# elybrand/quantized_neural_networks

Measured on NVIDIA B200. Metric: quantized weights/s, full-network GPFQ pass, higher is better.
Workload: dtype f64

## Files before the change

### quantized_neural_networks_b200/csrc/api.cu

```cuda
#include <math.h>
#include <stdarg.h>
#include <stdlib.h>

#include <algorithm>
#include <cmath>

#include "common.cuh"

int dense_gram_path(gpfq_ctx *, const float *, const float *, int64_t, int64_t, int64_t, const float *, int64_t,
                    int64_t, int64_t, const double *, const int *, const int *, int, double *, int64_t, int64_t,
                    gpfq_stats *, const double *G1_pre = nullptr, const double *G2_pre = nullptr, const double *d_scales = nullptr,
                    int64_t u0 = 0);
int dense_stream_path(gpfq_ctx *, const float *, const float *, int64_t, int64_t, int64_t, const float *, int64_t,
                      int64_t, int64_t, const double *, const int *, const int *, int, double *, int64_t, int64_t,
                      gpfq_stats *, const double *d_scales, int64_t u0);
int dense_gram_only(gpfq_ctx *, const float *, const float *, int64_t, int64_t, int64_t, double *, double *);
bool dense_gram_uses_i8(gpfq_ctx *, int64_t, int64_t, bool);
int conv_supported_kk(int kk);
int conv_pick_chunks(gpfq_ctx *, int64_t, int, int64_t *, int, bool, int64_t part_rows = 0);
bool conv_specialised_kk(int kk);
int conv_gram_stage(gpfq_ctx *, int, ConvPtrs, bool, int64_t, int, int, int64_t, double *, bool, int);
int conv_finalize_stage(gpfq_ctx *, const double *, int, int, int, bool, double *);
int conv_sweep_stage(gpfq_ctx *, int, const double *, const float *, double *, int64_t, int64_t, int64_t, int,
                     const double *, const int *, const int *, int, int64_t, const double *);
int im2col_stage(gpfq_ctx *, const float *, int64_t, int, int, int64_t, int64_t, int, int, int, int, int, int, int,
                 int, int, int, int, float *, int64_t);
int msq_stage(gpfq_ctx *, const void *, int, int64_t, const double *, int, int, double *, const double *, int64_t);
int nhwc9_plan(int, int, int, int, int, int, int, int, int *, int *);
int corr9_plan(int, int, int, int, int, int, int, int, int, int);
int corr9_pack_stage(gpfq_ctx *, const float *, int64_t, int, int, int64_t, int64_t, int, int, int64_t, int64_t, float *);
int corr9_pick_slots(gpfq_ctx *, int, bool, int64_t, int, int64_t, int);
int corr9_uses_strips(gpfq_ctx *, int);
int corr9_tensor_ok(const float *, const float *);
int conv_corr9_stage(gpfq_ctx *, const float *, const float *, bool, int64_t, int64_t, int64_t, int, int, int64_t, int64_t, int,
                     int, double *, int, int, int, double *, int, int, int);
int conv_corr9_assemble_stage(gpfq_ctx *, const double *, int, const double *, int, bool, int, int, double *);
int conv_gram9_nhwc_stage(gpfq_ctx *, const float *, const float *, bool, int64_t, int64_t, int, int, int64_t, int64_t, int,
                          int, int, int, int, int, int, int, double *, int);

int gpfq_fail(gpfq_ctx *ctx, int code, const char *fmt, ...) {
    char buf[1024];
    va_list ap;
    va_start(ap, fmt);
    vsnprintf(buf, sizeof(buf), fmt, ap);
    va_end(ap);
    if (ctx) ctx->err = buf;
    return code;
}

int gpfq_ws(gpfq_ctx *ctx, int slot, size_t bytes, void **out) {
    DevBuf &b = ctx->ws[slot];
    if (bytes == 0) bytes = 16;
    if (b.cap < bytes) {
        if (b.p) {
            CUDA_TRY(ctx, cudaStreamSynchronize(ctx->stream));
            CUDA_TRY(ctx, cudaStreamSynchronize(ctx->copy_stream));
            for (auto &s : ctx->aux_stream) if (s) CUDA_TRY(ctx, cudaStreamSynchronize(s));
            CUDA_TRY(ctx, cudaFree(b.p));
            b.p = nullptr;
            b.cap = 0;
        }
        size_t cap = (bytes + ((size_t)1 << 20) - 1) & ~(((size_t)1 << 20) - 1);
        cudaError_t e = cudaMalloc(&b.p, cap);
        if (e != cudaSuccess) {
            b.p = nullptr;
            cudaGetLastError();
            return gpfq_fail(ctx, GPFQ_ERR_OOM, "cudaMalloc of %zu bytes (workspace %d) failed: %s", cap, slot,
                             cudaGetErrorString(e));
        }
        b.cap = cap;
    }
    *out = b.p;
    return GPFQ_OK;
}

int gpfq_pinned(gpfq_ctx *ctx, int slot, size_t bytes, void **out) {
    DevBuf &b = ctx->pinned[slot];
    if (bytes == 0) bytes = 16;
    if (b.cap < bytes) {
        if (b.p) {
            CUDA_TRY(ctx, cudaStreamSynchronize(ctx->stream));
            CUDA_TRY(ctx, cudaFreeHost(b.p));
            b.p = nullptr;
            b.cap = 0;
        }
        cudaError_t e = cudaMallocHost(&b.p, bytes);
        if (e != cudaSuccess) {
            b.p = nullptr;
            cudaGetLastError();
            return gpfq_fail(ctx, GPFQ_ERR_OOM, "cudaMallocHost of %zu bytes failed: %s", bytes, cudaGetErrorString(e));
        }
        b.cap = bytes;
    }
    *out = b.p;
    return GPFQ_OK;
}

extern "C" int gpfq_version(void) { return GPFQ_VERSION; }

extern "C" int gpfq_create(int device, gpfq_ctx **out) {
    if (!out) return GPFQ_ERR_ARG;
    *out = nullptr;
    int ndev = 0;
    if (cudaGetDeviceCount(&ndev) != cudaSuccess || device < 0 || device >= ndev) {
        cudaGetLastError();
        return GPFQ_ERR_UNSUPPORTED;
    }
    cudaDeviceProp prop;
    if (cudaGetDeviceProperties(&prop, device) != cudaSuccess) return GPFQ_ERR_CUDA;
    if (prop.major != 10) return GPFQ_ERR_UNSUPPORTED;
    if (cudaSetDevice(device) != cudaSuccess) return GPFQ_ERR_CUDA;
    gpfq_ctx *ctx = new gpfq_ctx();
    ctx->device = device;
    ctx->sm_count = prop.multiProcessorCount;
    ctx->smem_optin = prop.sharedMemPerBlockOptin;
    bool ok = cudaStreamCreateWithFlags(&ctx->own_stream, cudaStreamNonBlocking) == cudaSuccess &&
              cudaStreamCreateWithFlags(&ctx->copy_stream, cudaStreamNonBlocking) == cudaSuccess;
    ctx->ring.resize(GPFQ_RING);
    for (auto &r : ctx->ring)
        for (int i = 0; ok && i < 8; ++i) ok = cudaEventCreate(&r.e[i]) == cudaSuccess;
    ctx->cur = &ctx->ring[0];
    for (int i = 0; ok && i < 4; ++i) ok = cudaEventCreateWithFlags(&ctx->ev_copy[i], cudaEventDisableTiming) == cudaSuccess;
    for (int i = 0; ok && i < 12; ++i) ok = cudaEventCreateWithFlags(&ctx->ev_chain[i], cudaEventDisableTiming) == cudaSuccess;
    for (int i = 0; ok && i < 8; ++i) ok = cudaStreamCreateWithFlags(&ctx->aux_stream[i], cudaStreamNonBlocking) == cudaSuccess;
    if (!ok) {
        delete ctx;
        return GPFQ_ERR_CUDA;
    }
    ctx->stream = ctx->own_stream;
    *out = ctx;
    return GPFQ_OK;
}

extern "C" int64_t gpfq_conv_partial_bytes(gpfq_ctx *ctx) { return ctx ? ctx->conv_part_bytes : 0; }

extern "C" int gpfq_trim(gpfq_ctx *ctx) {
    if (!ctx) return GPFQ_ERR_ARG;
    cudaSetDevice(ctx->device);
    cudaStreamSynchronize(ctx->stream);
    cudaStreamSynchronize(ctx->copy_stream);
    for (auto &s : ctx->aux_stream) if (s) cudaStreamSynchronize(s);
    for (auto &b : ctx->ws) {
        if (b.p) cudaFree(b.p);
        b.p = nullptr;
        b.cap = 0;
    }
    for (auto &b : ctx->pinned) {
        if (b.p) cudaFreeHost(b.p);
        b.p = nullptr;
        b.cap = 0;
    }
    ctx->alph_cache.clear();
    ctx->alph_used = 0;
    ctx->i8_oom_bytes = 0;
    return GPFQ_OK;
}

extern "C" void gpfq_destroy(gpfq_ctx *ctx) {
    if (!ctx) return;
    gpfq_trim(ctx);
    for (auto &r : ctx->ring)
        for (auto &e : r.e) if (e) cudaEventDestroy(e);
    for (auto &e : ctx->ev_copy) if (e) cudaEventDestroy(e);
    for (auto &e : ctx->ev_chain) if (e) cudaEventDestroy(e);
    for (auto &s : ctx->aux_stream) if (s) cudaStreamDestroy(s);
    if (ctx->own_stream) cudaStreamDestroy(ctx->own_stream);
    if (ctx->copy_stream) cudaStreamDestroy(ctx->copy_stream);
    delete ctx;
}

extern "C" const char *gpfq_last_error(const gpfq_ctx *ctx) { return ctx ? ctx->err.c_str() : "null context"; }

extern "C" int gpfq_set_option(gpfq_ctx *ctx, const char *key, int64_t value) {
    if (!ctx || !key) return GPFQ_ERR_ARG;
    ctx->err.clear();
    if (!strcmp(key, "gram_kernel")) {
        if (value < 0 || value > 2) return gpfq_fail(ctx, GPFQ_ERR_ARG, "gram_kernel must be 0, 1 or 2");
        ctx->gram_variant = (int)value;
    } else if (!strcmp(key, "i8_pairs_d")) {
        if (value != 0 && (value < 2 || value > 10)) return gpfq_fail(ctx, GPFQ_ERR_ARG, "i8_pairs_d must be 0 or 2..10");
        ctx->i8_pairs_d = (int)value;
    } else if (!strcmp(key, "corr_pack")) {
        if (value < 0 || value > 2) return gpfq_fail(ctx, GPFQ_ERR_ARG, "corr_pack must be 0, 1 or 2");
        ctx->corr_pack = (int)value;
    } else if (!strcmp(key, "corr_small")) {
        ctx->corr_direct_small = value != 0;
    } else if (!strcmp(key, "corr_rows")) {
        if (value != 0 && value != 4 && value != 6 && value != 8) return gpfq_fail(ctx, GPFQ_ERR_ARG, "corr_rows must be 0, 4, 6 or 8");
        ctx->corr_rb = (int)value;
    } else if (!strcmp(key, "corr_strip")) {
        if (value != 0 && value != 2) return gpfq_fail(ctx, GPFQ_ERR_ARG, "corr_strip must be 0 or 2");
        ctx->corr_strip = (int)value;
    } else if (!strcmp(key, "conv_kernel")) {
        if (value < 0 || value > 3) return gpfq_fail(ctx, GPFQ_ERR_ARG, "conv_kernel must be 0, 1, 2 or 3");
        ctx->conv_variant = (int)value;
    } else if (!strcmp(key, "sweep_outer")) {
        if (value < 0 || value > 3) return gpfq_fail(ctx, GPFQ_ERR_ARG, "sweep_outer must be 0, 1, 2 or 3");
        ctx->lowrank_variant = (int)value;
    } else if (!strcmp(key, "sweep_walk")) {
        if (value < 0 || value > 2) return gpfq_fail(ctx, GPFQ_ERR_ARG, "sweep_walk must be 0, 1 or 2");
        ctx->sweep_walk = (int)value;
    } else if (!strcmp(key, "sweep_i8")) {
        if (value < 0 || value > 2) return gpfq_fail(ctx, GPFQ_ERR_ARG, "sweep_i8 must be 0, 1 or 2");
        ctx->sweep_i8 = (int)value;
    } else {
        return gpfq_fail(ctx, GPFQ_ERR_ARG, "unknown option '%s'", key);
    }
    return GPFQ_OK;
}

extern "C" int gpfq_set_rounding(gpfq_ctx *ctx, int32_t mode, const uint64_t *seeds, int32_t n_seeds) {
    if (!ctx) return GPFQ_ERR_ARG;
    ctx->err.clear();
    if (mode == GPFQ_ROUND_NEAREST) {
        ctx->rounding = mode;
        ctx->seeds.clear();
        return GPFQ_OK;
    }
    if (mode != GPFQ_ROUND_STOCHASTIC) return gpfq_fail(ctx, GPFQ_ERR_ARG, "unknown rounding mode %d", mode);
    if (!seeds || n_seeds < 1) return gpfq_fail(ctx, GPFQ_ERR_ARG, "stochastic rounding needs n_seeds >= 1 seeds");
    ctx->rounding = mode;
    ctx->seeds.assign(seeds, seeds + n_seeds);
    return GPFQ_OK;
}

extern "C" int gpfq_set_l1_penalty(gpfq_ctx *ctx, const double *lambdas, int32_t n_lambdas) {
    if (!ctx) return GPFQ_ERR_ARG;
    ctx->err.clear();
    if (n_lambdas < 0 || (n_lambdas > 0 && !lambdas)) return gpfq_fail(ctx, GPFQ_ERR_ARG, "bad n_lambdas=%d", n_lambdas);
    for (int i = 0; i < n_lambdas; ++i)
        if (!std::isfinite(lambdas[i]) || !(lambdas[i] >= 0.0))
            return gpfq_fail(ctx, GPFQ_ERR_ARG, "L1 penalty %d must be finite and >= 0", i);
    ctx->l1.assign(lambdas, lambdas + n_lambdas);
    return GPFQ_OK;
}

extern "C" int gpfq_set_stream(gpfq_ctx *ctx, void *cuda_stream) {
    if (!ctx) return GPFQ_ERR_ARG;
    cudaStream_t next = cuda_stream ? (cudaStream_t)cuda_stream : ctx->own_stream;
    if (next != ctx->stream) {
        cudaSetDevice(ctx->device);
        if (cudaStreamSynchronize(ctx->stream) != cudaSuccess) cudaGetLastError();
        ctx->stream = next;
    }
    return GPFQ_OK;
}

struct Alphabets {
    const double *d_levels = nullptr;
    const int *d_koff = nullptr;
    const int *d_flags = nullptr;
    std::vector<int> h_koff, h_flags;
};

static int alphabet_is_equispaced(const double *a, int K) {
    if (K < 2) return 0;
    const double step = (a[K - 1] - a[0]) / (K - 1);
    if (!(step > 0.0) || !std::isfinite(step)) return 0;
    for (int k = 0; k < K; ++k)
        if (!(fabs(a[k] - (a[0] + k * step)) <= 0.01 * step)) return 0;
    return 1;
}

static int upload_alphabets(gpfq_ctx *ctx, const double *alphabets, const int32_t *K, int n_alph, Alphabets *out) {
    if (!alphabets || !K || n_alph < 1 || n_alph > 1024) return gpfq_fail(ctx, GPFQ_ERR_ARG, "bad alphabet arguments");
    out->h_koff.assign(n_alph + 1, 0);
    for (int a = 0; a < n_alph; ++a) {
        if (K[a] < 1 || K[a] > GPFQ_MAX_K)
            return gpfq_fail(ctx, GPFQ_ERR_ARG, "alphabet %d has %d levels (supported: 1..%d)", a, K[a], GPFQ_MAX_K);
        out->h_koff[a + 1] = out->h_koff[a] + K[a];
    }
    const size_t nlev = out->h_koff[n_alph];
    const size_t lev_bytes = nlev * sizeof(double);
    out->h_flags.assign(n_alph, 0);
    for (int a = 0; a < n_alph; ++a) out->h_flags[a] = alphabet_is_equispaced(alphabets + out->h_koff[a], K[a]);
    const size_t koff_bytes = (n_alph + 1) * sizeof(int);
    const size_t bytes = (lev_bytes + koff_bytes + n_alph * sizeof(int) + 15) & ~(size_t)15;
    std::vector<char> blob(bytes, 0);
    memcpy(blob.data(), alphabets, lev_bytes);
    memcpy(blob.data() + lev_bytes, out->h_koff.data(), koff_bytes);
    memcpy(blob.data() + lev_bytes + koff_bytes, out->h_flags.data(), n_alph * sizeof(int));
    const size_t cap = (size_t)1 << 20;
    char *d = nullptr;
    GPFQ_TRY(gpfq_ws(ctx, WS_ALPH, cap, (void **)&d));
    const AlphEntry *hit = nullptr;
    for (const auto &e : ctx->alph_cache)
        if (e.blob.size() == bytes && memcmp(e.blob.data(), blob.data(), bytes) == 0) { hit = &e; break; }
    if (!hit) {
        if (bytes > cap) return gpfq_fail(ctx, GPFQ_ERR_ARG, "alphabet table too large");
        if (ctx->alph_used + bytes > cap || ctx->alph_cache.size() >= 256) {
            CUDA_TRY(ctx, cudaStreamSynchronize(ctx->stream));
            ctx->alph_cache.clear();
            ctx->alph_used = 0;
        }
        ctx->alph_cache.emplace_back();
        AlphEntry &e = ctx->alph_cache.back();
        e.blob.swap(blob);
        e.off = ctx->alph_used;
        ctx->alph_used += bytes;
        CUDA_TRY(ctx, cudaMemcpyAsync(d + e.off, e.blob.data(), bytes, cudaMemcpyHostToDevice, ctx->stream));
        hit = &e;
    }
    ctx->h_alph = alphabets;
    ctx->h_koff = out->h_koff.data();
    ctx->h_flags = out->h_flags.data();
    out->d_levels = reinterpret_cast<const double *>(d + hit->off);
    out->d_koff = reinterpret_cast<const int *>(d + hit->off + lev_bytes);
    out->d_flags = reinterpret_cast<const int *>(d + hit->off + lev_bytes + koff_bytes);
    return GPFQ_OK;
}

static int check_scales(gpfq_ctx *ctx, const double *scales, int n_alph, int64_t n, int64_t lds) {
    if (!scales) return gpfq_fail(ctx, GPFQ_ERR_ARG, "NULL scales");
    for (int a = 0; a < n_alph; ++a)
        for (int64_t j = 0; j < n; ++j) {
            const double v = scales[a * lds + j];
            if (!(v >= 0.0) || !std::isfinite(v))
                return gpfq_fail(ctx, GPFQ_ERR_ARG, "scale %lld of alphabet %d is %g (scales must be finite and >= 0)", (long long)j, a, v);
        }
    return GPFQ_OK;
}

static int upload_scales(gpfq_ctx *ctx, const double *scales, int n_alph, int64_t n, int64_t lds, const double **out) {
    double *d = nullptr;
    GPFQ_TRY(gpfq_ws(ctx, WS_SCALES, (size_t)n_alph * n * sizeof(double), (void **)&d));
    CUDA_TRY(ctx, cudaMemcpy2DAsync(d, n * sizeof(double), scales, lds * sizeof(double), n * sizeof(double), n_alph,
                                    cudaMemcpyHostToDevice, ctx->stream));
    *out = d;
    return GPFQ_OK;
}

static int check_rounding(gpfq_ctx *ctx, const double *alphabets, const int32_t *K, int n_alph) {
    if (ctx->rounding != GPFQ_ROUND_STOCHASTIC || !alphabets || !K) return GPFQ_OK;
    if ((size_t)n_alph > ctx->seeds.size())
        return gpfq_fail(ctx, GPFQ_ERR_ARG, "%d alphabets but %zu stochastic-rounding seeds", n_alph, ctx->seeds.size());
    int64_t off = 0;
    for (int a = 0; a < n_alph; ++a) {
        if (K[a] < 1 || K[a] > GPFQ_MAX_K) return GPFQ_OK;
        for (int k = 0; k < K[a]; ++k) {
            const double v = alphabets[off + k];
            if (!std::isfinite(v) || (k > 0 && !(alphabets[off + k - 1] <= v)))
                return gpfq_fail(ctx, GPFQ_ERR_ARG, "stochastic rounding: alphabet %d must be non-decreasing and finite", a);
        }
        off += K[a];
    }
    return GPFQ_OK;
}

static int stage_seeds(gpfq_ctx *ctx, int n_alph) {
    ctx->d_seeds = nullptr;
    if (ctx->rounding != GPFQ_ROUND_STOCHASTIC || ctx->gram_only_out) return GPFQ_OK;
    uint64_t *d = nullptr;
    GPFQ_TRY(gpfq_ws(ctx, WS_SEEDS, (size_t)n_alph * sizeof(uint64_t), (void **)&d));
    CUDA_TRY(ctx, cudaMemcpyAsync(d, ctx->seeds.data(), (size_t)n_alph * sizeof(uint64_t), cudaMemcpyHostToDevice, ctx->stream));
    ctx->d_seeds = d;
    return GPFQ_OK;
}

static int check_l1(gpfq_ctx *ctx, int n_alph) {
    if (ctx->l1.empty() || (size_t)n_alph <= ctx->l1.size()) return GPFQ_OK;
    return gpfq_fail(ctx, GPFQ_ERR_ARG, "%d alphabets but %zu L1 penalties", n_alph, ctx->l1.size());
}

static int stage_l1(gpfq_ctx *ctx, int n_alph) {
    ctx->d_l1 = nullptr;
    if (ctx->l1.empty() || ctx->gram_only_out) return GPFQ_OK;
    double *d = nullptr;
    GPFQ_TRY(gpfq_ws(ctx, WS_L1_LAMBDA, (size_t)n_alph * sizeof(double), (void **)&d));
    CUDA_TRY(ctx, cudaMemcpyAsync(d, ctx->l1.data(), (size_t)n_alph * sizeof(double), cudaMemcpyHostToDevice, ctx->stream));
    ctx->d_l1 = d;
    return GPFQ_OK;
}

cudaError_t gpfq_record(gpfq_ctx *ctx, int which, cudaStream_t s) {
    ctx->cur->rec[which] = true;
    return cudaEventRecord(ctx->cur->e[which], s);
}

static void begin_call(gpfq_ctx *ctx, int kind) {
    ctx->cur = &ctx->ring[ctx->calls % GPFQ_RING];
    ctx->calls++;
    for (bool &r : ctx->cur->rec) r = false;
    ctx->cur->kind = kind;
    ctx->cur->st = gpfq_stats{};
    ctx->launches = 0;
}

static float ev_ms(const CallRecord &r, int a, int b) {
    float ms = 0.f;
    if (!r.rec[a] || !r.rec[b]) return 0.f;
    if (cudaEventElapsedTime(&ms, r.e[a], r.e[b]) != cudaSuccess) { cudaGetLastError(); return 0.f; }
    return ms;
}

static void fill_times(CallRecord &r) {
    gpfq_stats &st = r.st;
    st.ms_total = ev_ms(r, 0, 1);
    st.ms_h2d = ev_ms(r, 0, 5);
    if (r.kind == 1) {
        st.ms_stream = ev_ms(r, 2, 3);
        st.ms_d2h = ev_ms(r, 6, 1);
    } else {
        st.ms_gram = ev_ms(r, 2, 3);
        st.ms_sweep = ev_ms(r, 3, 4);
        st.ms_d2h = r.kind == 0 ? ev_ms(r, 6, 1) : ev_ms(r, 4, 1);
    }
}

static void end_call(gpfq_ctx *ctx, gpfq_stats *stats, bool synced) {
    CallRecord &r = *ctx->cur;
    if (stats) r.st = *stats;
    r.st.kernel_launches = ctx->launches;
    if (synced) fill_times(r);
    if (stats) *stats = r.st;
}

extern "C" int gpfq_query_stats(gpfq_ctx *ctx, int32_t calls_back, gpfq_stats *out) {
    if (!ctx || !out || calls_back < 0 || calls_back >= GPFQ_RING || calls_back >= ctx->calls) return GPFQ_ERR_ARG;
    CallRecord &r = ctx->ring[(ctx->calls - 1 - calls_back) % GPFQ_RING];
    fill_times(r);
    *out = r.st;
    return GPFQ_OK;
}

static int choose_dense_method(gpfq_ctx *ctx, uint32_t flags, int64_t N0, int64_t m, int64_t nj, bool same, int n_alph) {
    const uint32_t want = flags & GPFQ_METHOD_MASK;
    if (want != GPFQ_METHOD_AUTO) return (int)want;
    const double slots_per_s = 18.5e12 * 0.6;
    const bool u_in_regs = m <= 512 * 16;
    const double waves = ceil((double)nj / (double)ctx->sm_count);
    const double epv = ceil((double)m / 2048.0);
    double t_stream = n_alph * (3.0 * (double)m * N0 * nj / slots_per_s * (u_in_regs ? 1.0 : 4.0));
    const double t_steps = n_alph * waves * (double)N0 * (0.6e-6 + 0.37e-6 * (u_in_regs ? epv : 4.0 * epv));
    if (t_stream < t_steps) t_stream = t_steps;
    double t_gram_stage = (same ? 0.5 : 1.0) * (double)m * N0 * N0 / slots_per_s;
    if (dense_gram_uses_i8(ctx, N0, m, same)) {
        const double tile_area = (double)N0 * N0 * 0.5 + 192.0 * N0;
        t_gram_stage = (same ? 1.0 : 2.0) * (15.0 * 2.0 * tile_area * (double)m / 2.0e15 + 24.0 * N0 * (double)m / 5e12) + 4e-5;
    }
    const double sweep_rounds = ceil((double)ceil_div64(nj, 32) * n_alph / (2.0 * ctx->sm_count));
    double t_gram = t_gram_stage + n_alph * ((double)N0 * N0 * nj / slots_per_s) + sweep_rounds * (double)N0 * 0.6e-6;
    const double gram_bytes = (same ? 1.0 : 2.0) * 8.0 * N0 * N0;
    if (gram_bytes > 48e9) return GPFQ_METHOD_STREAM_FAST;
    return t_gram < t_stream ? GPFQ_METHOD_GRAM : GPFQ_METHOD_STREAM_FAST;
}

static int dense_layer(gpfq_ctx *ctx, const float *X, const float *Xq, int64_t ldx, int64_t N0, int64_t m, const float *W,
                       int64_t ldw, int64_t N1, int64_t j0, int64_t j1, const double *alphabets, const int32_t *K, int32_t n_alph,
                       double *Q_out, int64_t ldq, uint32_t flags, gpfq_stats *stats, const double *scales, int64_t lds,
                       int64_t ubase = 0) {
    if (!ctx) return GPFQ_ERR_ARG;
    ctx->err.clear();
    if (stats) memset(stats, 0, sizeof(*stats));
    if (!X || !W || !Q_out) return gpfq_fail(ctx, GPFQ_ERR_ARG, "NULL X, W or Q_out");
    if (N0 < 1 || m < 1 || N1 < 1 || ldx < m || ldw < N1 || ldq < N1 || j0 < 0 || j1 > N1 || j0 > j1)
        return gpfq_fail(ctx, GPFQ_ERR_ARG, "bad shape: N0=%lld m=%lld N1=%lld ldx=%lld ldw=%lld ldq=%lld j0=%lld j1=%lld",
                         (long long)N0, (long long)m, (long long)N1, (long long)ldx, (long long)ldw, (long long)ldq,
                         (long long)j0, (long long)j1);
    if (N0 > 2000000 || m > ((int64_t)1 << 40)) return gpfq_fail(ctx, GPFQ_ERR_ARG, "shape too large");
    if ((flags & GPFQ_NO_SYNC) && (flags & GPFQ_ALL_DEVICE) != GPFQ_ALL_DEVICE)
        return gpfq_fail(ctx, GPFQ_ERR_ARG, "GPFQ_NO_SYNC needs all-device pointers");
    const int64_t nj = j1 - j0;
    if (scales && n_alph >= 1) GPFQ_TRY(check_scales(ctx, scales + j0, n_alph, nj, lds));
    GPFQ_TRY(check_rounding(ctx, alphabets, K, n_alph));
    GPFQ_TRY(check_l1(ctx, n_alph));
    if (nj == 0) return GPFQ_OK;
    CUDA_TRY(ctx, cudaSetDevice(ctx->device));
    const bool same = (Xq == nullptr || Xq == X);
    cudaStream_t s = ctx->stream;
    const int method = choose_dense_method(ctx, flags, N0, m, nj, same, n_alph);
    begin_call(ctx, method == GPFQ_METHOD_GRAM ? 0 : 1);
    CUDA_TRY(ctx, gpfq_record(ctx, 0, s));

    Alphabets al;
    GPFQ_TRY(upload_alphabets(ctx, alphabets, K, n_alph, &al));
    GPFQ_TRY(stage_seeds(ctx, n_alph));
    GPFQ_TRY(stage_l1(ctx, n_alph));
    const double *d_scales = nullptr;
    if (scales) GPFQ_TRY(upload_scales(ctx, scales + j0, n_alph, nj, lds, &d_scales));

    const float *dX = X, *dXq = same ? X : Xq, *dW = W;
    int64_t dldx = ldx, dldw = ldw, dj0 = j0;
    if (!(flags & GPFQ_X_DEVICE)) {
        float *bx = nullptr, *bq = nullptr;
        GPFQ_TRY(gpfq_ws(ctx, WS_X, (size_t)N0 * m * sizeof(float), (void **)&bx));
        CUDA_TRY(ctx, cudaMemcpy2DAsync(bx, m * sizeof(float), X, ldx * sizeof(float), m * sizeof(float), N0,
                                        cudaMemcpyHostToDevice, s));
        dX = dXq = bx;
        if (!same) {
            GPFQ_TRY(gpfq_ws(ctx, WS_XQ, (size_t)N0 * m * sizeof(float), (void **)&bq));
            CUDA_TRY(ctx, cudaMemcpy2DAsync(bq, m * sizeof(float), Xq, ldx * sizeof(float), m * sizeof(float), N0,
                                            cudaMemcpyHostToDevice, s));
            dXq = bq;
        }
        dldx = m;
    }
    if (!(flags & GPFQ_W_DEVICE)) {
        float *bw = nullptr;
        GPFQ_TRY(gpfq_ws(ctx, WS_W, (size_t)N0 * nj * sizeof(float), (void **)&bw));
        CUDA_TRY(ctx, cudaMemcpy2DAsync(bw, nj * sizeof(float), W + j0, ldw * sizeof(float), nj * sizeof(float), N0,
                                        cudaMemcpyHostToDevice, s));
        dW = bw;
        dldw = nj;
        dj0 = 0;
    }
    double *dQ = Q_out;
    int64_t dldq = ldq, col0 = j0;
    if (!(flags & GPFQ_Q_DEVICE)) {
        GPFQ_TRY(gpfq_ws(ctx, WS_Q, (size_t)n_alph * N0 * nj * sizeof(double), (void **)&dQ));
        dldq = nj;
        col0 = 0;
    }
    CUDA_TRY(ctx, gpfq_record(ctx, 5, s));

    if (method == GPFQ_METHOD_GRAM)
        GPFQ_TRY(dense_gram_path(ctx, dX, dXq, dldx, N0, m, dW, dldw, dj0, nj, al.d_levels, al.d_koff, al.d_flags, n_alph, dQ,
                                 dldq, col0, stats, nullptr, nullptr, d_scales, ubase + j0));
    else {
        ctx->stream_literal = (method == GPFQ_METHOD_STREAM);
        GPFQ_TRY(dense_stream_path(ctx, dX, dXq, dldx, N0, m, dW, dldw, dj0, nj, al.d_levels, al.h_koff.data(),
                                   al.h_flags.data(), n_alph, dQ, dldq, col0, stats, d_scales, ubase + j0));
        if (stats) stats->method = method >> 4;
    }
    CUDA_TRY(ctx, gpfq_record(ctx, 6, s));
    if (!(flags & GPFQ_Q_DEVICE)) {
        for (int a = 0; a < n_alph; ++a)
            CUDA_TRY(ctx, cudaMemcpy2DAsync(Q_out + (int64_t)a * N0 * ldq + j0, ldq * sizeof(double),
                                            dQ + (int64_t)a * N0 * nj, nj * sizeof(double), nj * sizeof(double), N0,
                                            cudaMemcpyDeviceToHost, s));
    }
    CUDA_TRY(ctx, gpfq_record(ctx, 1, s));
    if (stats) stats->weights = N0 * nj * n_alph;
    const bool synced = !(flags & GPFQ_NO_SYNC);
    if (synced) CUDA_TRY(ctx, cudaStreamSynchronize(s));
    end_call(ctx, stats, synced);
    return GPFQ_OK;
}

extern "C" int gpfq_dense_layer(gpfq_ctx *ctx, const float *X, const float *Xq, int64_t ldx, int64_t N0, int64_t m,
                                const float *W, int64_t ldw, int64_t N1, int64_t j0, int64_t j1,
                                const double *alphabets, const int32_t *K, int32_t n_alph, double *Q_out,
                                int64_t ldq, uint32_t flags, gpfq_stats *stats) {
    return dense_layer(ctx, X, Xq, ldx, N0, m, W, ldw, N1, j0, j1, alphabets, K, n_alph, Q_out, ldq, flags, stats, nullptr, 0);
}

extern "C" int gpfq_dense_layer_scaled(gpfq_ctx *ctx, const float *X, const float *Xq, int64_t ldx, int64_t N0, int64_t m,
                                       const float *W, int64_t ldw, int64_t N1, int64_t j0, int64_t j1,
                                       const double *alphabets, const int32_t *K, int32_t n_alph, double *Q_out,
                                       int64_t ldq, uint32_t flags, gpfq_stats *stats, const double *scales) {
    if (ctx && !scales) return gpfq_fail(ctx, GPFQ_ERR_ARG, "NULL scales");
    return dense_layer(ctx, X, Xq, ldx, N0, m, W, ldw, N1, j0, j1, alphabets, K, n_alph, Q_out, ldq, flags, stats, scales, N1);
}

static int dense_layer_from_gram(gpfq_ctx *ctx, const double *G1, const double *G2, int64_t N0, const float *W, int64_t ldw,
                                 int64_t N1, int64_t j0, int64_t j1, const double *alphabets, const int32_t *K, int32_t n_alph,
                                 double *Q_out, int64_t ldq, uint32_t flags, gpfq_stats *stats, const double *scales) {
    if (!ctx) return GPFQ_ERR_ARG;
    ctx->err.clear();
    if (stats) memset(stats, 0, sizeof(*stats));
    if (!G2 || !W || !Q_out) return gpfq_fail(ctx, GPFQ_ERR_ARG, "NULL G2, W or Q_out");
    if (N0 < 1 || N1 < 1 || ldw < N1 || ldq < N1 || j0 < 0 || j1 > N1 || j0 > j1)
        return gpfq_fail(ctx, GPFQ_ERR_ARG, "bad shape: N0=%lld N1=%lld ldw=%lld ldq=%lld j0=%lld j1=%lld", (long long)N0,
                         (long long)N1, (long long)ldw, (long long)ldq, (long long)j0, (long long)j1);
    if (!(flags & GPFQ_X_DEVICE)) return gpfq_fail(ctx, GPFQ_ERR_ARG, "G1 / G2 must be device pointers (GPFQ_X_DEVICE)");
    if ((flags & GPFQ_NO_SYNC) && (flags & GPFQ_ALL_DEVICE) != GPFQ_ALL_DEVICE)
        return gpfq_fail(ctx, GPFQ_ERR_ARG, "GPFQ_NO_SYNC needs all-device pointers");
    const int64_t nj = j1 - j0;
    if (scales && n_alph >= 1) GPFQ_TRY(check_scales(ctx, scales + j0, n_alph, nj, N1));
    GPFQ_TRY(check_rounding(ctx, alphabets, K, n_alph));
    GPFQ_TRY(check_l1(ctx, n_alph));
    if (nj == 0) return GPFQ_OK;
    CUDA_TRY(ctx, cudaSetDevice(ctx->device));
    cudaStream_t s = ctx->stream;
    begin_call(ctx, 0);
    CUDA_TRY(ctx, gpfq_record(ctx, 0, s));
    Alphabets al;
    GPFQ_TRY(upload_alphabets(ctx, alphabets, K, n_alph, &al));
    GPFQ_TRY(stage_seeds(ctx, n_alph));
    GPFQ_TRY(stage_l1(ctx, n_alph));
    const double *d_scales = nullptr;
    if (scales) GPFQ_TRY(upload_scales(ctx, scales + j0, n_alph, nj, N1, &d_scales));
    const float *dW = W;
    int64_t dldw = ldw, dj0 = j0;
    if (!(flags & GPFQ_W_DEVICE)) {
        float *bw = nullptr;
        GPFQ_TRY(gpfq_ws(ctx, WS_W, (size_t)N0 * nj * sizeof(float), (void **)&bw));
        CUDA_TRY(ctx, cudaMemcpy2DAsync(bw, nj * sizeof(float), W + j0, ldw * sizeof(float), nj * sizeof(float), N0,
                                        cudaMemcpyHostToDevice, s));
        dW = bw;
        dldw = nj;
        dj0 = 0;
    }
    double *dQ = Q_out;
    int64_t dldq = ldq, col0 = j0;
    if (!(flags & GPFQ_Q_DEVICE)) {
        GPFQ_TRY(gpfq_ws(ctx, WS_Q, (size_t)n_alph * N0 * nj * sizeof(double), (void **)&dQ));
        dldq = nj;
        col0 = 0;
    }
    CUDA_TRY(ctx, gpfq_record(ctx, 5, s));
    GPFQ_TRY(dense_gram_path(ctx, nullptr, nullptr, 0, N0, 0, dW, dldw, dj0, nj, al.d_levels, al.d_koff, al.d_flags, n_alph,
                             dQ, dldq, col0, stats, (G1 == nullptr || G1 == G2) ? nullptr : G1, G2, d_scales, j0));
    CUDA_TRY(ctx, gpfq_record(ctx, 6, s));
    if (!(flags & GPFQ_Q_DEVICE)) {
        for (int a = 0; a < n_alph; ++a)
            CUDA_TRY(ctx, cudaMemcpy2DAsync(Q_out + (int64_t)a * N0 * ldq + j0, ldq * sizeof(double),
                                            dQ + (int64_t)a * N0 * nj, nj * sizeof(double), nj * sizeof(double), N0,
                                            cudaMemcpyDeviceToHost, s));
    }
    CUDA_TRY(ctx, gpfq_record(ctx, 1, s));
    if (stats) stats->weights = N0 * nj * n_alph;
    const bool synced = !(flags & GPFQ_NO_SYNC);
    if (synced) CUDA_TRY(ctx, cudaStreamSynchronize(s));
    end_call(ctx, stats, synced);
    return GPFQ_OK;
}

extern "C" int gpfq_dense_layer_from_gram(gpfq_ctx *ctx, const double *G1, const double *G2, int64_t N0, const float *W,
                                          int64_t ldw, int64_t N1, int64_t j0, int64_t j1, const double *alphabets,
                                          const int32_t *K, int32_t n_alph, double *Q_out, int64_t ldq, uint32_t flags,
                                          gpfq_stats *stats) {
    return dense_layer_from_gram(ctx, G1, G2, N0, W, ldw, N1, j0, j1, alphabets, K, n_alph, Q_out, ldq, flags, stats, nullptr);
}

extern "C" int gpfq_dense_layer_from_gram_scaled(gpfq_ctx *ctx, const double *G1, const double *G2, int64_t N0, const float *W,
                                                 int64_t ldw, int64_t N1, int64_t j0, int64_t j1, const double *alphabets,
                                                 const int32_t *K, int32_t n_alph, double *Q_out, int64_t ldq, uint32_t flags,
                                                 gpfq_stats *stats, const double *scales) {
    if (ctx && !scales) return gpfq_fail(ctx, GPFQ_ERR_ARG, "NULL scales");
    return dense_layer_from_gram(ctx, G1, G2, N0, W, ldw, N1, j0, j1, alphabets, K, n_alph, Q_out, ldq, flags, stats, scales);
}

extern "C" int gpfq_gram_matrices(gpfq_ctx *ctx, const float *X, const float *Xq, int64_t ldx, int64_t N0, int64_t m,
                                  double *G1_out, double *G2_out, uint32_t flags) {
    if (!ctx) return GPFQ_ERR_ARG;
    ctx->err.clear();
    if (!X || !G2_out || N0 < 1 || m < 1 || ldx < m) return gpfq_fail(ctx, GPFQ_ERR_ARG, "bad arguments");
    CUDA_TRY(ctx, cudaSetDevice(ctx->device));
    const bool same = (Xq == nullptr || Xq == X);
    cudaStream_t s = ctx->stream;
    const float *dX = X, *dXq = same ? X : Xq;
    int64_t dld = ldx;
    if (!(flags & GPFQ_X_DEVICE)) {
        float *bx = nullptr, *bq = nullptr;
        GPFQ_TRY(gpfq_ws(ctx, WS_X, (size_t)N0 * m * sizeof(float), (void **)&bx));
        CUDA_TRY(ctx, cudaMemcpy2DAsync(bx, m * sizeof(float), X, ldx * sizeof(float), m * sizeof(float), N0,
                                        cudaMemcpyHostToDevice, s));
        dX = dXq = bx;
        if (!same) {
            GPFQ_TRY(gpfq_ws(ctx, WS_XQ, (size_t)N0 * m * sizeof(float), (void **)&bq));
            CUDA_TRY(ctx, cudaMemcpy2DAsync(bq, m * sizeof(float), Xq, ldx * sizeof(float), m * sizeof(float), N0,
                                            cudaMemcpyHostToDevice, s));
            dXq = bq;
        }
        dld = m;
    }
    double *g1 = nullptr, *g2 = nullptr;
    if (flags & GPFQ_Q_DEVICE) {
        if (!same && !G1_out) return gpfq_fail(ctx, GPFQ_ERR_ARG, "G1_out is NULL but Xq != X");
        g2 = G2_out;
        g1 = same ? g2 : G1_out;
        CUDA_TRY(ctx, cudaMemsetAsync(g2, 0, (size_t)N0 * N0 * sizeof(double), s));
        if (!same) CUDA_TRY(ctx, cudaMemsetAsync(g1, 0, (size_t)N0 * N0 * sizeof(double), s));
        GPFQ_TRY(dense_gram_only(ctx, dX, dXq, dld, N0, m, g1, g2));
        if (same && G1_out && G1_out != G2_out)
            CUDA_TRY(ctx, cudaMemcpyAsync(G1_out, g2, (size_t)N0 * N0 * sizeof(double), cudaMemcpyDeviceToDevice, s));
        if (!(flags & GPFQ_NO_SYNC)) CUDA_TRY(ctx, cudaStreamSynchronize(s));
        return GPFQ_OK;
    }
    GPFQ_TRY(gpfq_ws(ctx, WS_G2, (size_t)N0 * N0 * sizeof(double), (void **)&g2));
    g1 = g2;
    if (!same) GPFQ_TRY(gpfq_ws(ctx, WS_G1, (size_t)N0 * N0 * sizeof(double), (void **)&g1));
    GPFQ_TRY(dense_gram_only(ctx, dX, dXq, dld, N0, m, g1, g2));
    CUDA_TRY(ctx, cudaMemcpyAsync(G2_out, g2, (size_t)N0 * N0 * sizeof(double), cudaMemcpyDeviceToHost, s));
    if (G1_out) CUDA_TRY(ctx, cudaMemcpyAsync(G1_out, g1, (size_t)N0 * N0 * sizeof(double), cudaMemcpyDeviceToHost, s));
    CUDA_TRY(ctx, cudaStreamSynchronize(s));
    return GPFQ_OK;
}

static int conv_copy_q_grouped(gpfq_ctx *ctx, double *Q_out, const double *dQ, int kk, int64_t Cg, int64_t F, int64_t Fg,
                               int64_t c0, int64_t n_ch, int n_alph, size_t wcount) {
    cudaStream_t s = ctx->stream;
    const size_t pitch = (size_t)F * sizeof(double);
    auto box = [&](int64_t r0, int64_t r1, int64_t g0, int64_t g1) -> int {
        if (r1 <= r0 || g1 <= g0) return GPFQ_OK;
        const size_t width = (size_t)(g1 - g0) * Fg * sizeof(double);
        for (int a = 0; a < n_alph; ++a) {
            const size_t off = (size_t)a * wcount + (size_t)r0 * F + (size_t)g0 * Fg;
            if (r0 == 0 && r1 == Cg) {
                CUDA_TRY(ctx, cudaMemcpy2DAsync(Q_out + off, pitch, dQ + off, pitch, width, (size_t)kk * Cg, cudaMemcpyDeviceToHost, s));
                continue;
            }
            for (int t = 0; t < kk; ++t) {
                const size_t o = off + (size_t)t * Cg * F;
                CUDA_TRY(ctx, cudaMemcpy2DAsync(Q_out + o, pitch, dQ + o, pitch, width, (size_t)(r1 - r0), cudaMemcpyDeviceToHost, s));
            }
        }
        return GPFQ_OK;
    };
    const int64_t c1 = c0 + n_ch, w0 = ceil_div64(c0, Cg), w1 = c1 / Cg;
    if (w0 > w1) return box(c0 % Cg, c1 % Cg, c0 / Cg, c0 / Cg + 1);
    GPFQ_TRY(box(c0 % Cg, Cg, c0 / Cg, w0));
    GPFQ_TRY(box(0, Cg, w0, w1));
    return box(0, c1 % Cg, w1, w1 + 1);
}

static int conv_finish(gpfq_ctx *ctx, int kk, const double *partial, int n_ch, int n_chunks, bool same,
                       const float *W, int64_t C, int64_t F, int64_t c0, const Alphabets &al, int n_alph,
                       double *Q_out, uint32_t flags, double *gram_ready = nullptr, int64_t groups = 1,
                       const double *d_scales = nullptr) {
    cudaStream_t s = ctx->stream;
    double *gram = gram_ready;
    if (!gram) {
        GPFQ_TRY(gpfq_ws(ctx, WS_CG, (size_t)n_ch * 2 * kk * kk * sizeof(double), (void **)&gram));
        GPFQ_TRY(conv_finalize_stage(ctx, partial, n_ch, n_chunks, kk, same, gram));
    }
    if (ctx->gram_only_out) {
        CUDA_TRY(ctx, cudaMemcpyAsync(ctx->gram_only_out, gram, (size_t)n_ch * 2 * kk * kk * sizeof(double),
                                      (flags & GPFQ_Q_DEVICE) ? cudaMemcpyDeviceToDevice : cudaMemcpyDeviceToHost, s));
        CUDA_TRY(ctx, gpfq_record(ctx, 4, s));
        return GPFQ_OK;
    }
    const float *dW = W;
    const int64_t Cg = C / groups;
    const size_t wcount = (size_t)kk * Cg * F;
    if (!(flags & GPFQ_W_DEVICE)) {
        float *bw = nullptr;
        GPFQ_TRY(gpfq_ws(ctx, WS_W, wcount * sizeof(float), (void **)&bw));
        CUDA_TRY(ctx, cudaMemcpyAsync(bw, W, wcount * sizeof(float), cudaMemcpyHostToDevice, s));
        dW = bw;
    }
    double *dQ = Q_out;
    if (!(flags & GPFQ_Q_DEVICE)) GPFQ_TRY(gpfq_ws(ctx, WS_Q, (size_t)n_alph * wcount * sizeof(double), (void **)&dQ));
    GPFQ_TRY(conv_sweep_stage(ctx, kk, gram, dW, dQ, C, F, c0, n_ch, al.d_levels, al.d_koff, al.d_flags, n_alph, groups, d_scales));
    CUDA_TRY(ctx, gpfq_record(ctx, 4, s));
    if (!(flags & GPFQ_Q_DEVICE) && groups > 1)
        return conv_copy_q_grouped(ctx, Q_out, dQ, kk, Cg, F, F / groups, c0, n_ch, n_alph, wcount);
    if (!(flags & GPFQ_Q_DEVICE)) {
        for (int a = 0; a < n_alph; ++a) {
            const size_t off = (size_t)a * wcount + (size_t)c0 * F;
            CUDA_TRY(ctx, cudaMemcpy2DAsync(Q_out + off, C * F * sizeof(double), dQ + off, C * F * sizeof(double),
                                            (size_t)n_ch * F * sizeof(double), kk, cudaMemcpyDeviceToHost, s));
        }
    }
    return GPFQ_OK;
}

static void conv_stats(gpfq_ctx *ctx, gpfq_stats *st, int kk, int64_t n, int64_t n_ch, int64_t F, bool same, int n_alph) {
    if (!st) return;
    st->weights = (int64_t)kk * n_ch * F * n_alph;
    st->method = GPFQ_METHOD_GRAM >> 4;
    st->bytes_algorithmic = (same ? 1 : 2) * 4LL * kk * n * n_ch;
    st->flops_algorithmic = (same ? 0 : 2LL * kk * kk * n * n_ch) + (int64_t)kk * (kk + 1) * n * n_ch;
    if (!conv_specialised_kk(kk)) st->flops_algorithmic = (same ? 1 : 2) * (int64_t)kk * (kk + 1) * n * n_ch;
}

static int conv_channels(gpfq_ctx *ctx, const float *const *Xp, const float *const *Xqp, int64_t n, int32_t kk, const float *W,
                         int64_t C, int64_t F, int64_t c0, int64_t n_ch, const double *alphabets, const int32_t *K,
                         int32_t n_alph, double *Q_out, uint32_t flags, gpfq_stats *stats, const double *scales) {
    if (!ctx) return GPFQ_ERR_ARG;
    ctx->err.clear();
    if (stats) memset(stats, 0, sizeof(*stats));
    if (!Xp || !W || !Q_out) return gpfq_fail(ctx, GPFQ_ERR_ARG, "NULL Xp, W or Q_out");
    if (n < 1 || kk < 1 || C < 1 || F < 1 || c0 < 0 || n_ch < 0 || c0 + n_ch > C || n_ch > 65535)
        return gpfq_fail(ctx, GPFQ_ERR_ARG, "bad shape: n=%lld kk=%d C=%lld F=%lld c0=%lld n_ch=%lld", (long long)n, kk,
                         (long long)C, (long long)F, (long long)c0, (long long)n_ch);
    if ((flags & GPFQ_NO_SYNC) && (flags & GPFQ_ALL_DEVICE) != GPFQ_ALL_DEVICE)
        return gpfq_fail(ctx, GPFQ_ERR_ARG, "GPFQ_NO_SYNC needs all-device pointers");
    if (scales && n_alph >= 1) GPFQ_TRY(check_scales(ctx, scales, n_alph, C * F, C * F));
    GPFQ_TRY(check_rounding(ctx, alphabets, K, n_alph));
    GPFQ_TRY(check_l1(ctx, n_alph));
    ctx->conv_part_bytes = 0;
    if (n_ch == 0) return GPFQ_OK;
    CUDA_TRY(ctx, cudaSetDevice(ctx->device));
    bool same = (Xqp == nullptr);
    if (!same) {
        same = true;
        for (int64_t i = 0; i < n_ch; ++i) same = same && (Xqp[i] == Xp[i] || Xqp[i] == nullptr);
    }
    for (int64_t i = 0; i < n_ch; ++i)
        if (!Xp[i] || (!same && !Xqp[i])) return gpfq_fail(ctx, GPFQ_ERR_ARG, "NULL patch pointer for channel %lld", (long long)i);

    if (!conv_supported_kk(kk)) {
        int64_t launches = 0;
        for (int64_t i = 0; i < n_ch; ++i) {
            const int64_t c = c0 + i;
            GPFQ_TRY(dense_layer(ctx, Xp[i], same ? Xp[i] : Xqp[i], n, kk, n, W + c * F, C * F, F, 0, F, alphabets, K, n_alph,
                                 Q_out + c * F, C * F, (flags & ~GPFQ_NO_SYNC) | GPFQ_METHOD_GRAM, stats,
                                 scales ? scales + c * F : nullptr, C * F, c * F));
            launches += stats ? stats->kernel_launches : 0;
        }
        if (stats) { stats->kernel_launches = (int)launches; stats->weights = (int64_t)kk * n_ch * F * n_alph; }
        return GPFQ_OK;
    }

    cudaStream_t s = ctx->stream;
    begin_call(ctx, 2);
    CUDA_TRY(ctx, gpfq_record(ctx, 0, s));
    Alphabets al;
    GPFQ_TRY(upload_alphabets(ctx, alphabets, K, n_alph, &al));
    GPFQ_TRY(stage_seeds(ctx, n_alph));
    GPFQ_TRY(stage_l1(ctx, n_alph));
    const double *d_scales = nullptr;
    if (scales) GPFQ_TRY(upload_scales(ctx, scales, n_alph, C * F, C * F, &d_scales));

    bool vec_ok = n % 4 == 0;
    if (flags & GPFQ_X_DEVICE)
        for (int64_t i = 0; i < n_ch; ++i)
            vec_ok = vec_ok && ((uintptr_t)Xp[i] % 16 == 0) && (same || (uintptr_t)Xqp[i] % 16 == 0);
    int64_t chunk_cols = 0;
    const int n_chunks = conv_pick_chunks(ctx, n, (int)n_ch, &chunk_cols, kk, vec_ok);
    double *partial = nullptr;
    ctx->conv_part_bytes = (int64_t)n_ch * n_chunks * 2 * kk * kk * (int64_t)sizeof(double);
    GPFQ_TRY(gpfq_ws(ctx, WS_CPART, (size_t)ctx->conv_part_bytes, (void **)&partial));
    const float **d_ptrs = nullptr;
    GPFQ_TRY(gpfq_ws(ctx, WS_PTRS, (size_t)2 * n_ch * sizeof(float *), (void **)&d_ptrs));
    std::vector<const float *> h_ptrs(2 * n_ch);
    const size_t ch_bytes = (size_t)kk * n * sizeof(float);

    CUDA_TRY(ctx, gpfq_record(ctx, 2, s));
    if (flags & GPFQ_X_DEVICE) {
        for (int64_t i = 0; i < n_ch; ++i) {
            h_ptrs[i] = Xp[i];
            h_ptrs[n_ch + i] = same ? Xp[i] : Xqp[i];
        }
        CUDA_TRY(ctx, cudaMemcpyAsync(d_ptrs, h_ptrs.data(), h_ptrs.size() * sizeof(float *), cudaMemcpyHostToDevice, s));
        ConvPtrs p{d_ptrs, d_ptrs + n_ch};
        GPFQ_TRY(conv_gram_stage(ctx, kk, p, same, n, (int)n_ch, n_chunks, chunk_cols, partial, vec_ok, n_chunks));
    } else {
        const size_t per_ch = ch_bytes * (same ? 1 : 2);
        const size_t budget = (size_t)6 << 30;
        int64_t bch = (int64_t)std::max<size_t>(1, budget / per_ch);
        bch = std::min<int64_t>(bch, n_ch);
        if (bch * 2 > n_ch && n_ch >= 2) bch = (n_ch + 1) / 2;
        float *buf[2] = {nullptr, nullptr};
        GPFQ_TRY(gpfq_ws(ctx, WS_PATCH_A, (size_t)bch * per_ch, (void **)&buf[0]));
        GPFQ_TRY(gpfq_ws(ctx, WS_PATCH_B, (size_t)bch * per_ch, (void **)&buf[1]));
        CUDA_TRY(ctx, cudaEventRecord(ctx->ev_copy[2], s));
        CUDA_TRY(ctx, cudaStreamWaitEvent(ctx->copy_stream, ctx->ev_copy[2], 0));
        int bi = 0;
        for (int64_t b0 = 0; b0 < n_ch; b0 += bch, ++bi) {
            const int64_t nb = std::min<int64_t>(bch, n_ch - b0);
            float *dst = buf[bi & 1];
            if (bi >= 2) CUDA_TRY(ctx, cudaStreamWaitEvent(ctx->copy_stream, ctx->ev_copy[bi & 1], 0));
            for (int64_t i = 0; i < nb; ++i) {
                float *dx = dst + (size_t)i * (per_ch / sizeof(float));
                CUDA_TRY(ctx, cudaMemcpyAsync(dx, Xp[b0 + i], ch_bytes, cudaMemcpyHostToDevice, ctx->copy_stream));
                h_ptrs[b0 + i] = dx;
                h_ptrs[n_ch + b0 + i] = dx;
                if (!same) {
                    float *dq = dx + (size_t)kk * n;
                    CUDA_TRY(ctx, cudaMemcpyAsync(dq, Xqp[b0 + i], ch_bytes, cudaMemcpyHostToDevice, ctx->copy_stream));
                    h_ptrs[n_ch + b0 + i] = dq;
                }
            }
            CUDA_TRY(ctx, cudaEventRecord(ctx->ev_copy[3], ctx->copy_stream));
            CUDA_TRY(ctx, cudaStreamWaitEvent(s, ctx->ev_copy[3], 0));
            CUDA_TRY(ctx, cudaMemcpyAsync(d_ptrs + b0, h_ptrs.data() + b0, nb * sizeof(float *), cudaMemcpyHostToDevice, s));
            CUDA_TRY(ctx, cudaMemcpyAsync(d_ptrs + n_ch + b0, h_ptrs.data() + n_ch + b0, nb * sizeof(float *),
                                          cudaMemcpyHostToDevice, s));
            ConvPtrs p{d_ptrs + b0, d_ptrs + n_ch + b0};
            GPFQ_TRY(conv_gram_stage(ctx, kk, p, same, n, (int)nb, n_chunks, chunk_cols,
                                     partial + (size_t)b0 * n_chunks * 2 * kk * kk, vec_ok, n_chunks));
            CUDA_TRY(ctx, cudaEventRecord(ctx->ev_copy[bi & 1], s));
        }
    }
    CUDA_TRY(ctx, gpfq_record(ctx, 3, s));
    GPFQ_TRY(conv_finish(ctx, kk, partial, (int)n_ch, n_chunks, same, W, C, F, c0, al, n_alph, Q_out, flags, nullptr, 1, d_scales));
    CUDA_TRY(ctx, gpfq_record(ctx, 1, s));
    gpfq_stats local = {};
    conv_stats(ctx, stats ? stats : &local, kk, n, n_ch, F, same, n_alph);
    const bool synced = !(flags & GPFQ_NO_SYNC);
    if (synced) CUDA_TRY(ctx, cudaStreamSynchronize(s));
    end_call(ctx, stats ? stats : &local, synced);
    return GPFQ_OK;
}

extern "C" int gpfq_conv_channels(gpfq_ctx *ctx, const float *const *Xp, const float *const *Xqp, int64_t n,
                                  int32_t kk, const float *W, int64_t C, int64_t F, int64_t c0, int64_t n_ch,
                                  const double *alphabets, const int32_t *K, int32_t n_alph, double *Q_out,
                                  uint32_t flags, gpfq_stats *stats) {
    return conv_channels(ctx, Xp, Xqp, n, kk, W, C, F, c0, n_ch, alphabets, K, n_alph, Q_out, flags, stats, nullptr);
}

extern "C" int gpfq_conv_channels_scaled(gpfq_ctx *ctx, const float *const *Xp, const float *const *Xqp, int64_t n,
                                         int32_t kk, const float *W, int64_t C, int64_t F, int64_t c0, int64_t n_ch,
                                         const double *alphabets, const int32_t *K, int32_t n_alph, double *Q_out,
                                         uint32_t flags, gpfq_stats *stats, const double *scales) {
    if (ctx && !scales) return gpfq_fail(ctx, GPFQ_ERR_ARG, "NULL scales");
    return conv_channels(ctx, Xp, Xqp, n, kk, W, C, F, c0, n_ch, alphabets, K, n_alph, Q_out, flags, stats, scales);
}

static int conv_layer_nhwc(gpfq_ctx *ctx, const float *act, const float *actq, int64_t n_img, int64_t H, int64_t Wd, int64_t C,
                           int32_t kh, int32_t kw, int32_t sh, int32_t sw, int32_t rh, int32_t rw, int32_t padding_same,
                           const float *W, int64_t F, int64_t c0, int64_t n_ch, const double *alphabets, const int32_t *K,
                           int32_t n_alph, double *Q_out, uint32_t flags, gpfq_stats *stats, int64_t groups,
                           const double *scales) {
    if (!ctx) return GPFQ_ERR_ARG;
    ctx->err.clear();
    if (stats) memset(stats, 0, sizeof(*stats));
    if (!act || !W || !Q_out) return gpfq_fail(ctx, GPFQ_ERR_ARG, "NULL act, W or Q_out");
    if (n_img < 1 || H < 1 || Wd < 1 || C < 1 || F < 1 || kh < 1 || kw < 1 || sh < 1 || sw < 1 || rh < 1 || rw < 1 ||
        c0 < 0 || n_ch < 0 || c0 + n_ch > C || H > 65535 || Wd > 65535)
        return gpfq_fail(ctx, GPFQ_ERR_ARG, "bad conv geometry");
    if (groups < 1 || C % groups || F % groups)
        return gpfq_fail(ctx, GPFQ_ERR_ARG, "bad groups=%lld for C=%lld, F=%lld", (long long)groups, (long long)C, (long long)F);
    const int64_t Cg = C / groups, Fg = F / groups;
    const int kk = kh * kw;
    if (scales && n_alph >= 1) GPFQ_TRY(check_scales(ctx, scales, n_alph, Cg * F, Cg * F));
    if (!ctx->gram_only_out) GPFQ_TRY(check_rounding(ctx, alphabets, K, n_alph));
    if (!ctx->gram_only_out) GPFQ_TRY(check_l1(ctx, n_alph));
    ctx->conv_part_bytes = 0;
    if (n_ch == 0) return GPFQ_OK;
    const int keh = (kh - 1) * rh + 1, kew = (kw - 1) * rw + 1;
    int Ho, Wo, pt = 0, pl = 0;
    if (padding_same) {
        Ho = (int)((H + sh - 1) / sh);
        Wo = (int)((Wd + sw - 1) / sw);
        const int64_t ph = std::max<int64_t>((int64_t)(Ho - 1) * sh + keh - H, 0);
        const int64_t pw = std::max<int64_t>((int64_t)(Wo - 1) * sw + kew - Wd, 0);
        pt = (int)(ph / 2);
        pl = (int)(pw / 2);
    } else {
        if (H < keh || Wd < kew) return gpfq_fail(ctx, GPFQ_ERR_ARG, "VALID padding: input smaller than the kernel");
        Ho = (int)((H - keh) / sh + 1);
        Wo = (int)((Wd - kew) / sw + 1);
    }
    const int64_t n = n_img * Ho * Wo;
    CUDA_TRY(ctx, cudaSetDevice(ctx->device));
    cudaStream_t s = ctx->stream;
    const bool same = (actq == nullptr || actq == act);
    if (!conv_supported_kk(kk)) {
        if (ctx->gram_only_out) return gpfq_fail(ctx, GPFQ_ERR_UNSUPPORTED, "kernel %dx%d has no Gram-only (image split) path", kh, kw);
        const size_t abytes_g = (size_t)n_img * H * Wd * C * sizeof(float);
        const float *gA = act, *gAq = same ? act : actq;
        if (!(flags & GPFQ_X_DEVICE)) {
            float *ba = nullptr, *bq = nullptr;
            GPFQ_TRY(gpfq_ws(ctx, WS_ACT_A, abytes_g, (void **)&ba));
            CUDA_TRY(ctx, cudaMemcpyAsync(ba, act, abytes_g, cudaMemcpyHostToDevice, s));
            gA = gAq = ba;
            if (!same) {
                GPFQ_TRY(gpfq_ws(ctx, WS_ACT_B, abytes_g, (void **)&bq));
                CUDA_TRY(ctx, cudaMemcpyAsync(bq, actq, abytes_g, cudaMemcpyHostToDevice, s));
                gAq = bq;
            }
        }
        float *pa = nullptr, *pq = nullptr;
        GPFQ_TRY(gpfq_ws(ctx, WS_PATCH_A, (size_t)kk * n * sizeof(float), (void **)&pa));
        pq = pa;
        if (!same) GPFQ_TRY(gpfq_ws(ctx, WS_PATCH_B, (size_t)kk * n * sizeof(float), (void **)&pq));
        int64_t launches = 0;
        for (int64_t i = 0; i < n_ch; ++i) {
            const int64_t c = c0 + i;
            GPFQ_TRY(im2col_stage(ctx, gA, n_img, (int)H, (int)Wd, C, c, 1, kh, kw, sh, sw, rh, rw, pt, pl, Ho, Wo, pa, (int64_t)kk * n));
            if (!same)
                GPFQ_TRY(im2col_stage(ctx, gAq, n_img, (int)H, (int)Wd, C, c, 1, kh, kw, sh, sw, rh, rw, pt, pl, Ho, Wo, pq, (int64_t)kk * n));
            const int64_t off = (c % Cg) * F + (c / Cg) * Fg;
            GPFQ_TRY(dense_layer(ctx, pa, same ? pa : pq, n, kk, n, W + off, Cg * F, Fg, 0, Fg, alphabets, K, n_alph, Q_out + off,
                                 Cg * F, ((flags & ~GPFQ_NO_SYNC) | GPFQ_X_DEVICE | GPFQ_METHOD_GRAM), stats,
                                 scales ? scales + off : nullptr, Cg * F, off));
            launches += (stats ? stats->kernel_launches : 0) + (same ? 1 : 2);
        }
        if (stats) { stats->kernel_launches = (int)launches; stats->weights = (int64_t)kk * n_ch * Fg * n_alph; }
        return GPFQ_OK;
    }
    begin_call(ctx, 2);
    CUDA_TRY(ctx, gpfq_record(ctx, 0, s));
    Alphabets al;
    GPFQ_TRY(upload_alphabets(ctx, alphabets, K, n_alph, &al));
    GPFQ_TRY(stage_seeds(ctx, n_alph));
    GPFQ_TRY(stage_l1(ctx, n_alph));
    const double *d_scales = nullptr;
    if (scales) GPFQ_TRY(upload_scales(ctx, scales, n_alph, Cg * F, Cg * F, &d_scales));
    const float *dA = act, *dAq = same ? act : actq;
    const size_t img_elems = (size_t)H * Wd * C;
    const size_t abytes = (size_t)n_img * img_elems * sizeof(float);
    const bool host_act = !(flags & GPFQ_X_DEVICE);
    int64_t ipc = n_img;
    if (host_act) {
        const size_t target = (size_t)96 << 20;
        ipc = (int64_t)std::max<size_t>(1, target / (img_elems * sizeof(float)));
        ipc = std::max<int64_t>(ipc, ceil_div64(n_img, 32));
        ipc = std::min<int64_t>(ceil_div64(ipc, 4) * 4, n_img);
    }
    int n_ic = (int)ceil_div64(n_img, ipc);
    if (host_act && !conv_specialised_kk(kk)) {
        const int64_t max_ic = std::max<int64_t>(1, CONV_PART_LIMIT / (n_ch * 2 * kk * kk * (int64_t)sizeof(double)));
        if (n_ic > max_ic) {
            ipc = std::min<int64_t>(ceil_div64(ceil_div64(n_img, max_ic), 4) * 4, n_img);
            n_ic = (int)ceil_div64(n_img, ipc);
        }
    }
    if (host_act) {
        float *ba = nullptr, *bq = nullptr;
        GPFQ_TRY(gpfq_ws(ctx, WS_ACT_A, abytes, (void **)&ba));
        dA = dAq = ba;
        if (!same) {
            GPFQ_TRY(gpfq_ws(ctx, WS_ACT_B, abytes, (void **)&bq));
            dAq = bq;
        }
    }
    CUDA_TRY(ctx, gpfq_record(ctx, 5, s));
    const int corr_rb = ctx->conv_variant == 0 ? corr9_plan(kh, kw, sh, sw, rh, rw, padding_same, (int)H, (int)Wd, ctx->corr_rb) : 0;
    const bool corr_direct = C >= 32 && C % 4 == 0 && n_ch >= 8 && (H * Wd >= 128 || (H * Wd >= 64 && corr9_uses_strips(ctx, (int)Wd)));
    int corr_G = 1;
    if (corr_rb && !(C >= 32 && C % 4 == 0) && (H * Wd >= 4096 || (H * Wd >= 1024 && corr9_uses_strips(ctx, (int)Wd))) && ctx->corr_pack != 2) {
        int g = 32, a = (int)(n_ch % 32);
        while (a) { const int t = g % a; g = a; a = t; }
        corr_G = 32 / g;
        const double packed = (double)ceil_div64(n_img, corr_G) * corr_G * H * Wd * n_ch * sizeof(float) * (same ? 1 : 2);
        if (corr_G * n_ch > 4096 || packed > 32e9) corr_G = 1;
    }
    if (ctx->corr_pack == 1 && corr_rb) {
        int g = 32, a = (int)(n_ch % 32);
        while (a) { const int t = g % a; g = a; a = t; }
        corr_G = 32 / g;
        if (corr_G == 1 || corr_G * n_ch > 4096) corr_G = (corr_G * n_ch > 4096) ? 1 : 2;
    }
    if (corr_rb && (corr_G > 1 || (corr_direct && ctx->corr_pack != 1) || (ctx->corr_direct_small && C >= 32 && C % 4 == 0 && n_ch >= 8)) &&
        corr9_tensor_ok(dA, dAq)) {
        const bool pack = corr_G > 1;
        const int64_t VC = pack ? (int64_t)corr_G * n_ch : C;
        const int vch = pack ? (int)VC : (int)n_ch;
        const int64_t vc0 = pack ? 0 : c0;
        int64_t cipc = ipc;
        if (pack) cipc = std::min<int64_t>(ceil_div64(cipc, corr_G) * corr_G, ceil_div64(n_img, corr_G) * corr_G);
        const int cn_ic = (int)ceil_div64(n_img, cipc);
        const int64_t units_per_chunk = pack ? cipc / corr_G : cipc;
        const int64_t units_total = pack ? ceil_div64(n_img, corr_G) : n_img;
        const int nbands = (int)ceil_div64(H - 2, corr_rb);
        const int per_ic = corr9_pick_slots(ctx, corr_rb, same, vc0, vch, units_per_chunk * nbands, (int)Wd);
        const int bper_ic = corr9_pick_slots(ctx, 1, same, vc0, vch, 2 * units_per_chunk, (int)Wd);
        const int slots = cn_ic * per_ic, bslots = cn_ic * bper_ic;
        double *partial = nullptr, *bpartial = nullptr, *gram = nullptr;
        float *pkA = nullptr, *pkQ = nullptr;
        const size_t part_bytes = (size_t)vch * slots * 78 * sizeof(double);
        const size_t bpart_bytes = (size_t)vch * bslots * 78 * sizeof(double);
        ctx->conv_part_bytes = (int64_t)part_bytes;
        GPFQ_TRY(gpfq_ws(ctx, WS_CPART, part_bytes, (void **)&partial));
        GPFQ_TRY(gpfq_ws(ctx, WS_CORR_B, bpart_bytes, (void **)&bpartial));
        GPFQ_TRY(gpfq_ws(ctx, WS_CG, (size_t)n_ch * 2 * kk * kk * sizeof(double), (void **)&gram));
        if (pack) {
            const size_t pk_bytes = (size_t)units_total * H * Wd * VC * sizeof(float);
            GPFQ_TRY(gpfq_ws(ctx, WS_PATCH_A, pk_bytes, (void **)&pkA));
            pkQ = pkA;
            if (!same) GPFQ_TRY(gpfq_ws(ctx, WS_PATCH_B, pk_bytes, (void **)&pkQ));
        }
        CUDA_TRY(ctx, cudaMemsetAsync(partial, 0, part_bytes, s));
        CUDA_TRY(ctx, cudaMemsetAsync(bpartial, 0, bpart_bytes, s));
        CUDA_TRY(ctx, gpfq_record(ctx, 2, s));
        if (host_act) {
            CUDA_TRY(ctx, cudaEventRecord(ctx->ev_copy[2], s));
            CUDA_TRY(ctx, cudaStreamWaitEvent(ctx->copy_stream, ctx->ev_copy[2], 0));
        }
        for (int ic = 0; ic < cn_ic; ++ic) {
            const int64_t img0 = (int64_t)ic * cipc;
            const int64_t imgs = std::min<int64_t>(cipc, n_img - img0);
            if (host_act) {
                const size_t off = (size_t)img0 * img_elems, bytes = (size_t)imgs * img_elems * sizeof(float);
                CUDA_TRY(ctx, cudaMemcpyAsync(const_cast<float *>(dA) + off, act + off, bytes, cudaMemcpyHostToDevice, ctx->copy_stream));
                if (!same)
                    CUDA_TRY(ctx, cudaMemcpyAsync(const_cast<float *>(dAq) + off, actq + off, bytes, cudaMemcpyHostToDevice, ctx->copy_stream));
                CUDA_TRY(ctx, cudaEventRecord(ctx->ev_copy[ic & 1], ctx->copy_stream));
                CUDA_TRY(ctx, cudaStreamWaitEvent(s, ctx->ev_copy[ic & 1], 0));
            }
            if (pack) {
                GPFQ_TRY(corr9_pack_stage(ctx, dA, n_img, (int)H, (int)Wd, C, c0, (int)n_ch, corr_G, img0, imgs, pkA));
                if (!same) GPFQ_TRY(corr9_pack_stage(ctx, dAq, n_img, (int)H, (int)Wd, C, c0, (int)n_ch, corr_G, img0, imgs, pkQ));
                GPFQ_TRY(conv_corr9_stage(ctx, pkA, pkQ, same, img0 / corr_G, ceil_div64(imgs, corr_G), units_total, (int)H, (int)Wd, VC,
                                          0, vch, corr_rb, partial, slots, ic * per_ic, per_ic, bpartial, bslots, ic * bper_ic, bper_ic));
            } else {
                GPFQ_TRY(conv_corr9_stage(ctx, dA, dAq, same, img0, imgs, n_img, (int)H, (int)Wd, C, c0, (int)n_ch, corr_rb, partial, slots,
                                          ic * per_ic, per_ic, bpartial, bslots, ic * bper_ic, bper_ic));
            }
        }
        GPFQ_TRY(conv_corr9_assemble_stage(ctx, partial, slots, bpartial, bslots, same, (int)n_ch, pack ? corr_G : 1, gram));
        CUDA_TRY(ctx, gpfq_record(ctx, 3, s));
        GPFQ_TRY(conv_finish(ctx, kk, nullptr, (int)n_ch, 0, same, W, C, F, c0, al, n_alph, Q_out, flags, gram, groups, d_scales));
        CUDA_TRY(ctx, gpfq_record(ctx, 1, s));
        gpfq_stats local = {};
        gpfq_stats *st = stats ? stats : &local;
        conv_stats(ctx, st, kk, n, n_ch, Fg, same, n_alph);
        st->bytes_algorithmic = (same ? 1 : 2) * 4LL * n_img * H * Wd * n_ch;
        st->flops_algorithmic = (same ? 1 : 2) * 26LL * n_img * H * Wd * n_ch;
        st->gram_kernel = pack ? 5 : 4;
        const bool synced = !(flags & GPFQ_NO_SYNC);
        if (synced) CUDA_TRY(ctx, cudaStreamSynchronize(s));
        end_call(ctx, st, synced);
        return GPFQ_OK;
    }
    int planeP = 0, bandR = 0;
    if ((ctx->conv_variant == 0 || ctx->conv_variant == 3) && nhwc9_plan(kh, kw, sh, sw, rh, rw, Ho, Wo, &planeP, &bandR)) {
        const int64_t ctas = ceil_div64(n_ch, 8);
        int64_t per_ic = ceil_div64(4LL * 2 * ctx->sm_count, ctas * n_ic);
        per_ic = std::max<int64_t>(1, std::min<int64_t>(per_ic, ipc));
        const int slots = (int)(n_ic * per_ic);
        double *partial = nullptr;
        const size_t part_bytes = (size_t)ctas * 8 * slots * 2 * kk * kk * sizeof(double);
        ctx->conv_part_bytes = (int64_t)part_bytes;
        GPFQ_TRY(gpfq_ws(ctx, WS_CPART, part_bytes, (void **)&partial));
        CUDA_TRY(ctx, cudaMemsetAsync(partial, 0, part_bytes, s));
        CUDA_TRY(ctx, gpfq_record(ctx, 2, s));
        if (host_act) {
            CUDA_TRY(ctx, cudaEventRecord(ctx->ev_copy[2], s));
            CUDA_TRY(ctx, cudaStreamWaitEvent(ctx->copy_stream, ctx->ev_copy[2], 0));
        }
        for (int ic = 0; ic < n_ic; ++ic) {
            const int64_t img0 = (int64_t)ic * ipc;
            const int64_t imgs = std::min<int64_t>(ipc, n_img - img0);
            if (host_act) {
                const size_t off = (size_t)img0 * img_elems, bytes = (size_t)imgs * img_elems * sizeof(float);
                CUDA_TRY(ctx, cudaMemcpyAsync(const_cast<float *>(dA) + off, act + off, bytes, cudaMemcpyHostToDevice, ctx->copy_stream));
                if (!same)
                    CUDA_TRY(ctx, cudaMemcpyAsync(const_cast<float *>(dAq) + off, actq + off, bytes, cudaMemcpyHostToDevice, ctx->copy_stream));
                CUDA_TRY(ctx, cudaEventRecord(ctx->ev_copy[ic & 1], ctx->copy_stream));
                CUDA_TRY(ctx, cudaStreamWaitEvent(s, ctx->ev_copy[ic & 1], 0));
            }
            GPFQ_TRY(conv_gram9_nhwc_stage(ctx, dA, dAq, same, img0, imgs, (int)H, (int)Wd, C, c0, (int)n_ch, Ho, Wo, pt, pl,
                                           planeP, bandR, (int)per_ic, partial + (size_t)ic * per_ic * 2 * kk * kk, slots));
        }
        CUDA_TRY(ctx, gpfq_record(ctx, 3, s));
        GPFQ_TRY(conv_finish(ctx, kk, partial, (int)n_ch, slots, same, W, C, F, c0, al, n_alph, Q_out, flags, nullptr, groups, d_scales));
        CUDA_TRY(ctx, gpfq_record(ctx, 1, s));
        gpfq_stats local = {};
        gpfq_stats *st = stats ? stats : &local;
        conv_stats(ctx, st, kk, n, n_ch, Fg, same, n_alph);
        st->bytes_algorithmic = (same ? 1 : 2) * 4LL * n_img * H * Wd * n_ch;
        const bool synced = !(flags & GPFQ_NO_SYNC);
        if (synced) CUDA_TRY(ctx, cudaStreamSynchronize(s));
        end_call(ctx, st, synced);
        return GPFQ_OK;
    }
    const int64_t hw_out = (int64_t)Ho * Wo;
    const int64_t n_c = ipc * hw_out;
    bool vec_ok = n_c % 4 == 0 && ((n_img - (int64_t)(n_ic - 1) * ipc) * hw_out) % 4 == 0;
    int64_t chunk_cols = 0;
    const int n_chunks = conv_pick_chunks(ctx, n_c, (int)std::min<int64_t>(n_ch, 64), &chunk_cols, kk, vec_ok, n_ch * n_ic);
    const int slots = n_ic * n_chunks;
    double *partial = nullptr;
    const size_t part_bytes = (size_t)n_ch * slots * 2 * kk * kk * sizeof(double);
    ctx->conv_part_bytes = (int64_t)part_bytes;
        GPFQ_TRY(gpfq_ws(ctx, WS_CPART, part_bytes, (void **)&partial));
    if (n_ic > 1) CUDA_TRY(ctx, cudaMemsetAsync(partial, 0, part_bytes, s));
    const size_t ch_elems = (size_t)kk * n_c;
    const size_t per_ch = ch_elems * sizeof(float);
    const size_t budget = (size_t)8 << 30;
    int64_t bch = (int64_t)std::max<size_t>(1, budget / (per_ch * (same ? 1 : 2)));
    bch = std::min<int64_t>(bch, n_ch);
    float *pa = nullptr, *pq = nullptr;
    GPFQ_TRY(gpfq_ws(ctx, WS_PATCH_A, (size_t)bch * per_ch, (void **)&pa));
    if (!same) GPFQ_TRY(gpfq_ws(ctx, WS_PATCH_B, (size_t)bch * per_ch, (void **)&pq));
    const float **d_ptrs = nullptr;
    GPFQ_TRY(gpfq_ws(ctx, WS_PTRS, (size_t)2 * bch * n_ic * sizeof(float *), (void **)&d_ptrs));
    CUDA_TRY(ctx, gpfq_record(ctx, 2, s));
    if (host_act) {
        CUDA_TRY(ctx, cudaEventRecord(ctx->ev_copy[2], s));
        CUDA_TRY(ctx, cudaStreamWaitEvent(ctx->copy_stream, ctx->ev_copy[2], 0));
    }
    std::vector<const float *> h_ptrs((size_t)2 * bch * n_ic);
    for (int ic = 0; ic < n_ic; ++ic) {
        const int64_t img0 = (int64_t)ic * ipc;
        const int64_t imgs = std::min<int64_t>(ipc, n_img - img0);
        const int64_t n_this = imgs * hw_out;
        if (host_act) {
            const size_t off = (size_t)img0 * img_elems, bytes = (size_t)imgs * img_elems * sizeof(float);
            CUDA_TRY(ctx, cudaMemcpyAsync(const_cast<float *>(dA) + off, act + off, bytes, cudaMemcpyHostToDevice, ctx->copy_stream));
            if (!same)
                CUDA_TRY(ctx, cudaMemcpyAsync(const_cast<float *>(dAq) + off, actq + off, bytes, cudaMemcpyHostToDevice, ctx->copy_stream));
            CUDA_TRY(ctx, cudaEventRecord(ctx->ev_copy[ic & 1], ctx->copy_stream));
            CUDA_TRY(ctx, cudaStreamWaitEvent(s, ctx->ev_copy[ic & 1], 0));
        }
        const float **hp = h_ptrs.data() + (size_t)2 * bch * ic;
        for (int64_t i = 0; i < bch; ++i) {
            hp[i] = pa + (size_t)i * kk * n_this;
            hp[bch + i] = same ? hp[i] : pq + (size_t)i * kk * n_this;
        }
        const float **dp = d_ptrs + (size_t)2 * bch * ic;
        CUDA_TRY(ctx, cudaMemcpyAsync(dp, hp, (size_t)2 * bch * sizeof(float *), cudaMemcpyHostToDevice, s));
        const int chunks_this = (int)ceil_div64(n_this, chunk_cols);
        for (int64_t b0 = 0; b0 < n_ch; b0 += bch) {
            const int64_t nb = std::min<int64_t>(bch, n_ch - b0);
            GPFQ_TRY(im2col_stage(ctx, dA + (size_t)img0 * img_elems, imgs, (int)H, (int)Wd, C, c0 + b0, (int)nb, kh, kw, sh, sw,
                                  rh, rw, pt, pl, Ho, Wo, pa, (int64_t)kk * n_this));
            if (!same)
                GPFQ_TRY(im2col_stage(ctx, dAq + (size_t)img0 * img_elems, imgs, (int)H, (int)Wd, C, c0 + b0, (int)nb, kh, kw,
                                      sh, sw, rh, rw, pt, pl, Ho, Wo, pq, (int64_t)kk * n_this));
            ConvPtrs p{dp, dp + bch};
            GPFQ_TRY(conv_gram_stage(ctx, kk, p, same, n_this, (int)nb, chunks_this, chunk_cols,
                                     partial + ((size_t)b0 * slots + (size_t)ic * n_chunks) * 2 * kk * kk, vec_ok, slots));
        }
    }
    CUDA_TRY(ctx, gpfq_record(ctx, 3, s));
    GPFQ_TRY(conv_finish(ctx, kk, partial, (int)n_ch, slots, same, W, C, F, c0, al, n_alph, Q_out, flags, nullptr, groups, d_scales));
    CUDA_TRY(ctx, gpfq_record(ctx, 1, s));
    gpfq_stats local = {};
    conv_stats(ctx, stats ? stats : &local, kk, n, n_ch, Fg, same, n_alph);
    const bool synced = !(flags & GPFQ_NO_SYNC);
    if (synced) CUDA_TRY(ctx, cudaStreamSynchronize(s));
    end_call(ctx, stats ? stats : &local, synced);
    return GPFQ_OK;
}

extern "C" int gpfq_conv_layer_nhwc(gpfq_ctx *ctx, const float *act, const float *actq, int64_t n_img, int64_t H,
                                    int64_t Wd, int64_t C, int32_t kh, int32_t kw, int32_t sh, int32_t sw, int32_t rh,
                                    int32_t rw, int32_t padding_same, const float *W, int64_t F, int64_t c0,
                                    int64_t n_ch, const double *alphabets, const int32_t *K, int32_t n_alph,
                                    double *Q_out, uint32_t flags, gpfq_stats *stats) {
    return conv_layer_nhwc(ctx, act, actq, n_img, H, Wd, C, kh, kw, sh, sw, rh, rw, padding_same, W, F, c0, n_ch, alphabets, K,
                           n_alph, Q_out, flags, stats, 1, nullptr);
}

extern "C" int gpfq_conv_layer_nhwc_grouped(gpfq_ctx *ctx, const float *act, const float *actq, int64_t n_img, int64_t H,
                                            int64_t Wd, int64_t C, int32_t kh, int32_t kw, int32_t sh, int32_t sw, int32_t rh,
                                            int32_t rw, int32_t padding_same, const float *W, int64_t F, int64_t c0,
                                            int64_t n_ch, const double *alphabets, const int32_t *K, int32_t n_alph,
                                            double *Q_out, uint32_t flags, gpfq_stats *stats, int32_t groups) {
    return conv_layer_nhwc(ctx, act, actq, n_img, H, Wd, C, kh, kw, sh, sw, rh, rw, padding_same, W, F, c0, n_ch, alphabets, K,
                           n_alph, Q_out, flags, stats, groups, nullptr);
}

extern "C" int gpfq_conv_layer_nhwc_scaled(gpfq_ctx *ctx, const float *act, const float *actq, int64_t n_img, int64_t H,
                                           int64_t Wd, int64_t C, int32_t kh, int32_t kw, int32_t sh, int32_t sw, int32_t rh,
                                           int32_t rw, int32_t padding_same, const float *W, int64_t F, int64_t c0,
                                           int64_t n_ch, const double *alphabets, const int32_t *K, int32_t n_alph,
                                           double *Q_out, uint32_t flags, gpfq_stats *stats, int32_t groups,
                                           const double *scales) {
    if (ctx && !scales) return gpfq_fail(ctx, GPFQ_ERR_ARG, "NULL scales");
    return conv_layer_nhwc(ctx, act, actq, n_img, H, Wd, C, kh, kw, sh, sw, rh, rw, padding_same, W, F, c0, n_ch, alphabets, K,
                           n_alph, Q_out, flags, stats, groups, scales);
}

extern "C" int gpfq_conv_gram_nhwc(gpfq_ctx *ctx, const float *act, const float *actq, int64_t n_img, int64_t H, int64_t Wd,
                                   int64_t C, int32_t kh, int32_t kw, int32_t sh, int32_t sw, int32_t rh, int32_t rw,
                                   int32_t padding_same, int64_t c0, int64_t n_ch, double *gram_out, uint32_t flags) {
    if (!ctx) return GPFQ_ERR_ARG;
    if (!gram_out) return gpfq_fail(ctx, GPFQ_ERR_ARG, "NULL gram_out");
    static const double unit[2] = {-1.0, 1.0};
    static const int32_t two = 2;
    static const float w_dummy = 0.f;
    ctx->gram_only_out = gram_out;
    uint32_t f = flags | GPFQ_W_DEVICE;
    if ((f & GPFQ_ALL_DEVICE) != GPFQ_ALL_DEVICE) f &= ~GPFQ_NO_SYNC;
    const int rc = gpfq_conv_layer_nhwc(ctx, act, actq, n_img, H, Wd, C, kh, kw, sh, sw, rh, rw, padding_same, &w_dummy, 1, c0, n_ch,
                                        unit, &two, 1, gram_out, f, nullptr);
    ctx->gram_only_out = nullptr;
    return rc;
}

static int conv_layer_from_gram(gpfq_ctx *ctx, const double *gram, int32_t kk, const float *W, int64_t C, int64_t F, int64_t c0,
                                int64_t n_ch, const double *alphabets, const int32_t *K, int32_t n_alph, double *Q_out,
                                uint32_t flags, gpfq_stats *stats, int64_t groups, const double *scales) {
    if (!ctx) return GPFQ_ERR_ARG;
    ctx->err.clear();
    if (stats) memset(stats, 0, sizeof(*stats));
    if (!gram || !W || !Q_out) return gpfq_fail(ctx, GPFQ_ERR_ARG, "NULL gram, W or Q_out");
    if (!(flags & GPFQ_X_DEVICE)) return gpfq_fail(ctx, GPFQ_ERR_ARG, "gram must be a device pointer (GPFQ_X_DEVICE)");
    if (C < 1 || F < 1 || c0 < 0 || n_ch < 0 || c0 + n_ch > C) return gpfq_fail(ctx, GPFQ_ERR_ARG, "bad channel range");
    if (groups < 1 || C % groups || F % groups)
        return gpfq_fail(ctx, GPFQ_ERR_ARG, "bad groups=%lld for C=%lld, F=%lld", (long long)groups, (long long)C, (long long)F);
    if (!conv_supported_kk(kk)) return gpfq_fail(ctx, GPFQ_ERR_UNSUPPORTED, "kernel size kk=%d has no walk kernel", kk);
    if (scales && n_alph >= 1) GPFQ_TRY(check_scales(ctx, scales, n_alph, C / groups * F, C / groups * F));
    GPFQ_TRY(check_rounding(ctx, alphabets, K, n_alph));
    GPFQ_TRY(check_l1(ctx, n_alph));
    if (n_ch == 0) return GPFQ_OK;
    CUDA_TRY(ctx, cudaSetDevice(ctx->device));
    cudaStream_t s = ctx->stream;
    begin_call(ctx, 2);
    CUDA_TRY(ctx, gpfq_record(ctx, 0, s));
    Alphabets al;
    GPFQ_TRY(upload_alphabets(ctx, alphabets, K, n_alph, &al));
    GPFQ_TRY(stage_seeds(ctx, n_alph));
    GPFQ_TRY(stage_l1(ctx, n_alph));
    const double *d_scales = nullptr;
    if (scales) GPFQ_TRY(upload_scales(ctx, scales, n_alph, C / groups * F, C / groups * F, &d_scales));
    CUDA_TRY(ctx, gpfq_record(ctx, 5, s));
    CUDA_TRY(ctx, gpfq_record(ctx, 2, s));
    CUDA_TRY(ctx, gpfq_record(ctx, 3, s));
    GPFQ_TRY(conv_finish(ctx, kk, nullptr, (int)n_ch, 0, false, W, C, F, c0, al, n_alph, Q_out, flags, const_cast<double *>(gram),
                         groups, d_scales));
    CUDA_TRY(ctx, gpfq_record(ctx, 1, s));
    gpfq_stats local = {};
    gpfq_stats *st = stats ? stats : &local;
    st->weights = (int64_t)kk * n_ch * (F / groups) * n_alph;
    st->method = GPFQ_METHOD_GRAM >> 4;
    const bool synced = !(flags & GPFQ_NO_SYNC);
    if (synced) CUDA_TRY(ctx, cudaStreamSynchronize(s));
    end_call(ctx, st, synced);
    return GPFQ_OK;
}

extern "C" int gpfq_conv_layer_from_gram(gpfq_ctx *ctx, const double *gram, int32_t kk, const float *W, int64_t C, int64_t F,
                                         int64_t c0, int64_t n_ch, const double *alphabets, const int32_t *K, int32_t n_alph,
                                         double *Q_out, uint32_t flags, gpfq_stats *stats) {
    return conv_layer_from_gram(ctx, gram, kk, W, C, F, c0, n_ch, alphabets, K, n_alph, Q_out, flags, stats, 1, nullptr);
}

extern "C" int gpfq_conv_layer_from_gram_grouped(gpfq_ctx *ctx, const double *gram, int32_t kk, const float *W, int64_t C,
                                                 int64_t F, int64_t c0, int64_t n_ch, const double *alphabets, const int32_t *K,
                                                 int32_t n_alph, double *Q_out, uint32_t flags, gpfq_stats *stats,
                                                 int32_t groups) {
    return conv_layer_from_gram(ctx, gram, kk, W, C, F, c0, n_ch, alphabets, K, n_alph, Q_out, flags, stats, groups, nullptr);
}

extern "C" int gpfq_conv_layer_from_gram_scaled(gpfq_ctx *ctx, const double *gram, int32_t kk, const float *W, int64_t C,
                                                int64_t F, int64_t c0, int64_t n_ch, const double *alphabets, const int32_t *K,
                                                int32_t n_alph, double *Q_out, uint32_t flags, gpfq_stats *stats,
                                                int32_t groups, const double *scales) {
    if (ctx && !scales) return gpfq_fail(ctx, GPFQ_ERR_ARG, "NULL scales");
    return conv_layer_from_gram(ctx, gram, kk, W, C, F, c0, n_ch, alphabets, K, n_alph, Q_out, flags, stats, groups, scales);
}

static int round_elements(gpfq_ctx *ctx, const void *W, int is_f64, int64_t n, const double *alphabet, int32_t K,
                          double *Q_out, uint32_t flags, const double *scales = nullptr, int64_t n_units = 0) {
    if (!ctx) return GPFQ_ERR_ARG;
    ctx->err.clear();
    if (!W || !Q_out || n < 0) return gpfq_fail(ctx, GPFQ_ERR_ARG, "bad arguments");
    if (scales) {
        if (n_units < 1) return gpfq_fail(ctx, GPFQ_ERR_ARG, "n_units must be >= 1");
        GPFQ_TRY(check_scales(ctx, scales, 1, n_units, n_units));
    }
    GPFQ_TRY(check_rounding(ctx, alphabet, &K, 1));
    if (n == 0) return GPFQ_OK;
    CUDA_TRY(ctx, cudaSetDevice(ctx->device));
    begin_call(ctx, 2);
    cudaStream_t s = ctx->stream;
    Alphabets al;
    GPFQ_TRY(upload_alphabets(ctx, alphabet, &K, 1, &al));
    GPFQ_TRY(stage_seeds(ctx, 1));
    ctx->d_l1 = nullptr;
    const double *d_scales = nullptr;
    if (scales) GPFQ_TRY(upload_scales(ctx, scales, 1, n_units, n_units, &d_scales));
    const size_t esz = is_f64 ? sizeof(double) : sizeof(float);
    const void *dW = W;
    if (!(flags & GPFQ_W_DEVICE)) {
        void *bw = nullptr;
        GPFQ_TRY(gpfq_ws(ctx, WS_W, (size_t)n * esz, &bw));
        CUDA_TRY(ctx, cudaMemcpyAsync(bw, W, (size_t)n * esz, cudaMemcpyHostToDevice, s));
        dW = bw;
    }
    double *dQ = Q_out;
    if (!(flags & GPFQ_Q_DEVICE)) GPFQ_TRY(gpfq_ws(ctx, WS_Q, (size_t)n * sizeof(double), (void **)&dQ));
    GPFQ_TRY(msq_stage(ctx, dW, is_f64, n, al.d_levels, K, al.h_flags[0], dQ, d_scales, n_units));
    if (!(flags & GPFQ_Q_DEVICE))
        CUDA_TRY(ctx, cudaMemcpyAsync(Q_out, dQ, (size_t)n * sizeof(double), cudaMemcpyDeviceToHost, s));
    if (!(flags & GPFQ_NO_SYNC) || !(flags & GPFQ_Q_DEVICE)) CUDA_TRY(ctx, cudaStreamSynchronize(s));
    return GPFQ_OK;
}

extern "C" int gpfq_msq(gpfq_ctx *ctx, const float *W, int64_t n, const double *alphabet, int32_t K, double *Q_out,
                        uint32_t flags) {
    return round_elements(ctx, W, 0, n, alphabet, K, Q_out, flags);
}

extern "C" int gpfq_msq_scaled(gpfq_ctx *ctx, const float *W, int64_t n, const double *alphabet, int32_t K, const double *scales,
                               int64_t n_units, double *Q_out, uint32_t flags) {
    if (ctx && !scales) return gpfq_fail(ctx, GPFQ_ERR_ARG, "NULL scales");
    return round_elements(ctx, W, 0, n, alphabet, K, Q_out, flags, scales, n_units);
}

extern "C" int gpfq_bit_round(gpfq_ctx *ctx, const double *t, int64_t n, const double *alphabet, int32_t K,
                              double *out, uint32_t flags) {
    return round_elements(ctx, t, 1, n, alphabet, K, out, flags);
}
```

### quantized_neural_networks_b200/csrc/conv_corr.cu

```cuda
#include <cuda.h>

#include <algorithm>

#include "common.cuh"

namespace corr9 {
constexpr int ND = 13;
constexpr int WARPS = 4;
constexpr int WC = 5;
constexpr int REC = 6 * ND;
}

struct Corr9Geom {
    int H, W;
    int64_t c_first;
    int n_ch;
    int64_t img0, n_img;
    int slots;
    int y_first, y_last;
    int two_rows;
};

namespace corr9 {
__device__ __forceinline__ uint32_t smem_u32(const void *p) { return (uint32_t)__cvta_generic_to_shared(p); }
__device__ __forceinline__ void mbar_init(uint64_t *bar, int count) {
    asm volatile("mbarrier.init.shared::cta.b64 [%0], %1;\n" ::"r"(smem_u32(bar)), "r"(count));
}
__device__ __forceinline__ void mbar_expect_tx(uint64_t *bar, uint32_t bytes) {
    asm volatile("mbarrier.arrive.expect_tx.shared::cta.b64 _, [%0], %1;\n" ::"r"(smem_u32(bar)), "r"(bytes) : "memory");
}
__device__ __forceinline__ void mbar_wait(uint64_t *bar, uint32_t parity) {
    asm volatile(
        "{\n.reg .pred p;\nWAIT_%=:\n"
        "mbarrier.try_wait.parity.shared::cta.b64 p, [%0], %1;\n"
        "@p bra DONE_%=;\nbra WAIT_%=;\nDONE_%=:\n}\n" ::"r"(smem_u32(bar)), "r"(parity) : "memory");
}
__device__ __forceinline__ void tma_load_4d(void *dst, const CUtensorMap *map, uint64_t *bar, int c, int x, int y, int n) {
    asm volatile(
        "cp.async.bulk.tensor.4d.shared::cluster.global.mbarrier::complete_tx::bytes [%0], [%1, {%3, %4, %5, %6}], [%2];\n" ::"r"(
            smem_u32(dst)), "l"(map), "r"(smem_u32(bar)), "r"(c), "r"(x), "r"(y), "r"(n)
        : "memory");
}
template <int RB, bool CROSS>
struct Ring {
    static constexpr int NS = CROSS ? 2 : 3;
    static constexpr int B_FLOATS = (RB + 2) * WC * 32;
    static constexpr int A_FLOATS = CROSS ? RB * WC * 32 : 0;
    static constexpr int STAGE_FLOATS = B_FLOATS + A_FLOATS;
    static constexpr size_t WARP_BYTES = (size_t)NS * STAGE_FLOATS * sizeof(float);
    static constexpr size_t SMEM = WARPS * WARP_BYTES + WARPS * NS * sizeof(uint64_t);
};
}

template <int RB, bool CROSS>
__global__ void __launch_bounds__(corr9::WARPS * 32, RB <= 4 ? 3 : 2)
conv_corr9_tma_kernel(const __grid_constant__ CUtensorMap mapB, const __grid_constant__ CUtensorMap mapA, Corr9Geom gm,
                      double *__restrict__ partial, int slot_stride, int slot0) {
    using namespace corr9;
    using R = Ring<RB, CROSS>;
    constexpr int NS = R::NS;
    extern __shared__ __align__(128) unsigned char corr9_smem[];
    const int lane = threadIdx.x & 31, warp = threadIdx.x >> 5;
    const int slot = blockIdx.x * WARPS + warp;
    const int c0 = (int)(gm.c_first & ~(int64_t)3) + (int)blockIdx.y * 32;
    const int chl = c0 + lane - (int)gm.c_first;
    const bool chok = chl >= 0 && chl < gm.n_ch;
    float *ring = reinterpret_cast<float *>(corr9_smem + warp * R::WARP_BYTES);
    uint64_t *bars = reinterpret_cast<uint64_t *>(corr9_smem + WARPS * R::WARP_BYTES) + warp * NS;
    if (lane == 0) {
#pragma unroll
        for (int s = 0; s < NS; ++s) mbar_init(&bars[s], 1);
        asm volatile("fence.mbarrier_init.release.cluster;\n" ::: "memory");
    }
    __syncwarp();
    const int W = gm.W;
    const int nrows = gm.y_last - gm.y_first + 1;
    const int nbands = gm.two_rows ? 1 : (nrows + RB - 1) / RB;
    const int64_t ntasks = gm.two_rows ? gm.n_img : gm.n_img * nbands;
    const int64_t t_first = gm.two_rows ? slot / 2 : slot, t_step = gm.two_rows ? gm.slots / 2 : gm.slots;
    const int nstages = (W + 2 + WC - 1) / WC;
    double *rec = partial + ((size_t)(chok ? chl : 0) * slot_stride + slot0 + slot) * REC + (CROSS ? 0 : 3 * ND);
    uint32_t it = 0;
    double acc[ND];
#pragma unroll
    for (int d = 0; d < ND; ++d) acc[d] = 0.0;

    const int step_img = (int)(gm.two_rows ? t_step : t_step / nbands), step_band = gm.two_rows ? 0 : (int)(t_step % nbands);
    const int img_first = (int)(gm.img0 + (gm.two_rows ? t_first : t_first / nbands));
    const int band_first = gm.two_rows ? 0 : (int)(t_first % nbands);
    const int row_fixed = (slot & 1) ? gm.y_last : gm.y_first;
    int64_t ptask = t_first;
    int pk = 0, pimg = img_first, pband = band_first;
    uint32_t ppos = 0;
    auto produce = [&]() {
        if (ptask < ntasks) {
            if (lane == 0) {
                const int py0 = gm.two_rows ? row_fixed : gm.y_first + pband * RB;
                const int s = (int)(ppos % NS);
                float *dst = ring + s * R::STAGE_FLOATS;
                mbar_expect_tx(&bars[s], (uint32_t)(R::STAGE_FLOATS * sizeof(float)));
                tma_load_4d(dst, &mapB, &bars[s], c0, pk * WC, py0 - 2, pimg);
                if (CROSS) tma_load_4d(dst + R::B_FLOATS, &mapA, &bars[s], c0, pk * WC - 2, py0, pimg);
            }
            ++ppos;
            if (++pk == nstages) {
                pk = 0;
                ptask += t_step;
                pimg += step_img;
                pband += step_band;
                if (pband >= nbands) { pband -= nbands; ++pimg; }
            }
        }
    };
#pragma unroll
    for (int p = 0; p < NS - 1; ++p) produce();

    int cband = band_first;
    for (int64_t task = t_first; task < ntasks; task += t_step) {
        const int y0 = gm.two_rows ? row_fixed : gm.y_first + cband * RB;
        cband += step_band;
        if (cband >= nbands) cband -= nbands;
        unsigned rowmask = 0;
#pragma unroll
        for (int i = 0; i < RB; ++i) rowmask |= (y0 + i <= gm.y_last) ? (1u << i) : 0u;
        const bool allrows = rowmask == (1u << RB) - 1u;
        double win[RB + 2][5];
        double ac[RB];
        (void)ac;
#pragma unroll
        for (int r = 0; r < RB + 2; ++r)
#pragma unroll
            for (int c = 0; c < 5; ++c) win[r][c] = 0.0;
        for (int k = 0; k < nstages; ++k) {
            __syncwarp();
            produce();
            const uint32_t pos = it + k;
            const int s = (int)(pos % NS);
            mbar_wait(&bars[s], (pos / NS) & 1u);
            const float *tb = ring + s * R::STAGE_FLOATS + lane;
            const float *ta = tb + R::B_FLOATS;
            if (allrows && k >= 1 && k * WC + WC - 1 <= W) {
#pragma unroll
                for (int ph = 0; ph < WC; ++ph) {
#pragma unroll
                    for (int r = 0; r < RB + 2; ++r) win[r][ph] = (double)tb[(r * WC + ph) * 32];
                    if (CROSS) {
#pragma unroll
                        for (int i = 0; i < RB; ++i) ac[i] = (double)ta[(i * WC + ph) * 32];
                    }
#pragma unroll
                    for (int i = 0; i < RB; ++i) {
                        const double a = CROSS ? ac[i] : win[i + 2][(ph + 3) % 5];
#pragma unroll
                        for (int dy = 0; dy < 2; ++dy)
#pragma unroll
                            for (int dx = 0; dx < 5; ++dx)
                                acc[dy * 5 + dx] = fma(a, win[i + dy][(ph + 1 + dx) % 5], acc[dy * 5 + dx]);
#pragma unroll
                        for (int dx = 0; dx < 3; ++dx)
                            acc[10 + dx] = fma(a, win[i + 2][(ph + 1 + dx) % 5], acc[10 + dx]);
                    }
                }
            } else {
                float rawb[RB + 2], rawa[RB];
                (void)rawa;
                auto fetch = [&](int ph) {
#pragma unroll
                    for (int r = 0; r < RB + 2; ++r) rawb[r] = tb[(r * WC + ph) * 32];
                    if (CROSS) {
#pragma unroll
                        for (int i = 0; i < RB; ++i) rawa[i] = ta[(i * WC + ph) * 32];
                    }
                };
                fetch(0);
#pragma unroll
                for (int ph = 0; ph < WC; ++ph) {
                    const int cx = k * WC + ph;
                    if (cx < W + 2) {
#pragma unroll
                        for (int r = 0; r < RB + 2; ++r) win[r][ph] = (double)rawb[r];
                        if (CROSS) {
#pragma unroll
                            for (int i = 0; i < RB; ++i) ac[i] = (double)rawa[i];
                        }
                        if (ph + 1 < WC) fetch(ph + 1);
                        if (cx >= 2) {
                            double e[ND];
#pragma unroll
                            for (int d = 0; d < ND; ++d) e[d] = 0.0;
#pragma unroll
                            for (int i = 0; i < RB; ++i) {
                                double a = CROSS ? ac[i] : win[i + 2][(ph + 3) % 5];
                                a = (rowmask >> i) & 1u ? a : 0.0;
#pragma unroll
                                for (int dy = 0; dy < 2; ++dy)
#pragma unroll
                                    for (int dx = 0; dx < 5; ++dx)
                                        e[dy * 5 + dx] = fma(a, win[i + dy][(ph + 1 + dx) % 5], e[dy * 5 + dx]);
#pragma unroll
                                for (int dx = 0; dx < 3; ++dx)
                                    e[10 + dx] = fma(a, win[i + 2][(ph + 1 + dx) % 5], e[10 + dx]);
                            }
                            if (cx == 2 || cx == W + 1) {
                                if (chok) {
                                    double *o = rec + (cx == 2 ? 0 : 2 * ND);
#pragma unroll
                                    for (int d = 0; d < ND; ++d) atomicAdd(o + d, e[d]);
                                }
                            } else {
#pragma unroll
                                for (int d = 0; d < ND; ++d) acc[d] += e[d];
                            }
                        }
                    }
                }
            }
        }
        it += (uint32_t)nstages;
    }
    if (chok) {
#pragma unroll
        for (int d = 0; d < ND; ++d) rec[ND + d] = acc[d];
    }
}


namespace corr9s {
using corr9::ND;
using corr9::REC;
constexpr int WARPS = 4;
template <int RB> struct Boxes { static constexpr int NS = RB == 1 ? 2 : 1; };
template <int SW, int RB, bool CROSS>
struct Cfg {
    static constexpr int BW = SW + 4;
    static constexpr int WIN_FLOATS = (RB + 2) * BW * 32;
    static constexpr int CTR_FLOATS = CROSS ? RB * SW * 32 : 0;
    static constexpr int STAGE_FLOATS = WIN_FLOATS + CTR_FLOATS;
    static constexpr int NS = Boxes<RB>::NS;
    static constexpr size_t WARP_BYTES = (size_t)NS * STAGE_FLOATS * sizeof(float);
    static constexpr size_t SMEM = WARPS * WARP_BYTES + WARPS * NS * sizeof(uint64_t);
};
}

template <int SW, int RB, bool CROSS>
__global__ void __launch_bounds__(corr9s::WARPS * 32)
conv_corr9_strip_kernel(const __grid_constant__ CUtensorMap mapWin, const __grid_constant__ CUtensorMap mapCtr, Corr9Geom gm,
                        double *__restrict__ partial, int slot_stride, int slot0) {
    using namespace corr9s;
    using corr9::mbar_expect_tx;
    using corr9::mbar_init;
    using corr9::mbar_wait;
    using corr9::tma_load_4d;
    using C = Cfg<SW, RB, CROSS>;
    constexpr int BW = C::BW, NS = C::NS;
    extern __shared__ __align__(128) unsigned char corr9_smem[];
    const int lane = threadIdx.x & 31, warp = threadIdx.x >> 5;
    const int slot = blockIdx.x * WARPS + warp;
    const int c0 = (int)(gm.c_first & ~(int64_t)3) + (int)blockIdx.y * 32;
    const int chl = c0 + lane - (int)gm.c_first;
    const bool chok = chl >= 0 && chl < gm.n_ch;
    float *ring = reinterpret_cast<float *>(corr9_smem + warp * C::WARP_BYTES);
    uint64_t *bars = reinterpret_cast<uint64_t *>(corr9_smem + WARPS * C::WARP_BYTES) + warp * NS;
    if (lane == 0) {
#pragma unroll
        for (int s = 0; s < NS; ++s) mbar_init(&bars[s], 1);
        asm volatile("fence.mbarrier_init.release.cluster;\n" ::: "memory");
    }
    __syncwarp();
    const int nstrips = gm.W / SW;
    const int nrows = gm.y_last - gm.y_first + 1;
    const int nbands = gm.two_rows ? 1 : (nrows + RB - 1) / RB;
    const int per_img = nbands * nstrips;
    const int64_t ntasks = gm.n_img * per_img;
    const int64_t t_first = gm.two_rows ? slot / 2 : slot, t_step = gm.two_rows ? gm.slots / 2 : gm.slots;
    const int row_fixed = (slot & 1) ? gm.y_last : gm.y_first;
    const int step_img = (int)(t_step / per_img), step_in = (int)(t_step % per_img);
    auto fetch = [&](int img, int in, uint32_t pos) {
        const int band = in / nstrips, strip = in - band * nstrips;
        const int y0 = gm.two_rows ? row_fixed : gm.y_first + band * RB, x0 = strip * SW;
        const int s = (int)(pos % NS);
        float *dst = ring + s * C::STAGE_FLOATS;
        mbar_expect_tx(&bars[s], (uint32_t)(C::STAGE_FLOATS * sizeof(float)));
        tma_load_4d(dst, &mapWin, &bars[s], c0, x0 - 2, y0 - 2, img);
        if (CROSS) tma_load_4d(dst + C::WIN_FLOATS, &mapCtr, &bars[s], c0, x0, y0, img);
    };
    double acc[ND], accF[ND], accL[ND];
#pragma unroll
    for (int d = 0; d < ND; ++d) acc[d] = accF[d] = accL[d] = 0.0;
    int img = (int)(gm.img0 + t_first / per_img), in = (int)(t_first % per_img);
    if (t_first < ntasks && lane == 0) fetch(img, in, 0);
    uint32_t pos = 0;
    for (int64_t task = t_first; task < ntasks; task += t_step, ++pos) {
        int nimg = img + step_img, nin = in + step_in;
        if (nin >= per_img) { nin -= per_img; ++nimg; }
        if (NS > 1) {
            __syncwarp();
            if (task + t_step < ntasks && lane == 0) fetch(nimg, nin, pos + 1);
        }
        const int band = in / nstrips, strip = in - band * nstrips;
        const int y0 = gm.two_rows ? row_fixed : gm.y_first + band * RB;
        const bool left_edge = strip == 0, right_edge = strip == nstrips - 1;
        unsigned rowmask = 0;
#pragma unroll
        for (int i = 0; i < RB; ++i) rowmask |= (y0 + i <= gm.y_last) ? (1u << i) : 0u;
        const int s = (int)(pos % NS);
        mbar_wait(&bars[s], (pos / NS) & 1u);
        const float *tb = ring + s * C::STAGE_FLOATS + lane;
        const float *ta = tb + C::WIN_FLOATS;
        double win[RB + 2][6];
        double ctr[RB], ctr_n[RB];
        (void)ctr;
        (void)ctr_n;
#pragma unroll
        for (int bc = 0; bc < 5; ++bc)
#pragma unroll
            for (int r = 0; r < RB + 2; ++r) win[r][bc] = (double)tb[(r * BW + bc) * 32];
        if (CROSS) {
#pragma unroll
            for (int i = 0; i < RB; ++i) ctr[i] = (double)ta[(i * SW) * 32];
        }
#pragma unroll
        for (int p = 0; p < SW; ++p) {
            const bool edge = p == 0 || p == SW - 1;
            double e[ND];
            if (edge) {
#pragma unroll
                for (int d = 0; d < ND; ++d) e[d] = 0.0;
            }
#pragma unroll
            for (int i = 0; i < RB; ++i) {
                double a = CROSS ? ctr[i] : win[i + 2][(p + 2) % 6];
                a = (rowmask >> i) & 1u ? a : 0.0;
                if (edge) {
#pragma unroll
                    for (int dy = 0; dy < 2; ++dy)
#pragma unroll
                        for (int dx = 0; dx < 5; ++dx) e[dy * 5 + dx] = fma(a, win[i + dy][(p + dx) % 6], e[dy * 5 + dx]);
#pragma unroll
                    for (int dx = 0; dx < 3; ++dx) e[10 + dx] = fma(a, win[i + 2][(p + dx) % 6], e[10 + dx]);
                } else {
#pragma unroll
                    for (int dy = 0; dy < 2; ++dy)
#pragma unroll
                        for (int dx = 0; dx < 5; ++dx) acc[dy * 5 + dx] = fma(a, win[i + dy][(p + dx) % 6], acc[dy * 5 + dx]);
#pragma unroll
                    for (int dx = 0; dx < 3; ++dx) acc[10 + dx] = fma(a, win[i + 2][(p + dx) % 6], acc[10 + dx]);
                }
                if (p + 5 < BW) {
                    win[i][(p + 5) % 6] = (double)tb[(i * BW + p + 5) * 32];
                    if (i + RB < RB + 2) win[i + RB][(p + 5) % 6] = (double)tb[((i + RB) * BW + p + 5) * 32];
                    if (RB == 1) win[2][(p + 5) % 6] = (double)tb[(2 * BW + p + 5) * 32];
                }
                if (CROSS && p + 1 < SW) ctr_n[i] = (double)ta[(i * SW + p + 1) * 32];
            }
            if (CROSS) {
#pragma unroll
                for (int i = 0; i < RB; ++i) ctr[i] = ctr_n[i];
            }
            if (edge) {
                const bool first = p == 0 && left_edge, last = p == SW - 1 && right_edge;
#pragma unroll
                for (int d = 0; d < ND; ++d) {
                    accF[d] += first ? e[d] : 0.0;
                    accL[d] += last ? e[d] : 0.0;
                    acc[d] += (first || last) ? 0.0 : e[d];
                }
            }
        }
        if (NS == 1) {
            __syncwarp();
            if (task + t_step < ntasks && lane == 0) fetch(nimg, nin, pos + 1);
        }
        img = nimg;
        in = nin;
    }
    if (chok) {
        double *rec = partial + ((size_t)chl * slot_stride + slot0 + slot) * REC + (CROSS ? 0 : 3 * ND);
#pragma unroll
        for (int d = 0; d < ND; ++d) {
            rec[d] = accF[d];
            rec[ND + d] = acc[d];
            rec[2 * ND + d] = accL[d];
        }
    }
}

__global__ void __launch_bounds__(1024)
conv_corr9_assemble_kernel(const double *__restrict__ partial, int slots, const double *__restrict__ rpartial, int rslots,
                           int same, int n_ch, int G, double *__restrict__ gram) {
    using namespace corr9;
    constexpr int NV = 2 * 9 * ND, NP = 4;
    __shared__ double S[2][3][3][ND];
    __shared__ double P[NP][NV];
    const int ch = blockIdx.x, tid = threadIdx.x;
    const int e = tid % 256, part = tid / 256;
    if (e < NV) {
        const int d = e % ND, cc = (e / ND) % 3, rc = (e / (3 * ND)) % 3, pass = e / (9 * ND);
        const int off = (pass * 3 + cc) * ND + d;
        const int n = rc == 1 ? slots : (rslots - (rc == 0 ? 0 : 1) + 1) / 2;
        const size_t stride = rc == 1 ? REC : 2 * REC;
        double t0 = 0.0, t1 = 0.0, t2 = 0.0, t3 = 0.0;
        for (int g = 0; g < G; ++g) {
            const size_t vch = (size_t)g * n_ch + ch;
            const double *src = rc == 1 ? partial + vch * slots * REC + off
                                        : rpartial + (vch * rslots + (rc == 0 ? 0 : 1)) * REC + off;
            int s = part * 4;
#pragma unroll 2
            for (; s + 4 <= n; s += 4 * NP) {
                t0 += src[(size_t)s * stride];
                t1 += src[(size_t)(s + 1) * stride];
                t2 += src[(size_t)(s + 2) * stride];
                t3 += src[(size_t)(s + 3) * stride];
            }
            if (s < n) {
                t0 += src[(size_t)s * stride];
                if (s + 1 < n) t1 += src[(size_t)(s + 1) * stride];
                if (s + 2 < n) t2 += src[(size_t)(s + 2) * stride];
            }
        }
        P[part][e] = (t0 + t1) + (t2 + t3);
    }
    __syncthreads();
    if (tid < NV) {
        const int d = tid % ND, cc = (tid / ND) % 3, rc = (tid / (3 * ND)) % 3, pass = tid / (9 * ND);
        S[pass][rc][cc][d] = (P[0][tid] + P[1][tid]) + (P[2][tid] + P[3][tid]);
    }
    __syncthreads();
    for (int e2 = tid; e2 < 162; e2 += blockDim.x) {
        const int which = e2 / 81, t = (e2 % 81) / 9, s = e2 % 9;
        double v = 0.0;
        if (s <= t) {
            const int ar = t / 3, ac = t % 3, dy = s / 3 - ar, dx = s % 3 - ac;
            const int id = dy < 0 ? (dy + 2) * 5 + dx + 2 : 12 + dx;
            const int pass = (which == 0 && !same) ? 0 : 1;
            const int r_lo = ar == 2 ? 1 : 0, r_hi = ar == 0 ? 1 : 2, c_lo = ac == 2 ? 1 : 0, c_hi = ac == 0 ? 1 : 2;
            for (int rc = r_lo; rc <= r_hi; ++rc)
                for (int cc = c_lo; cc <= c_hi; ++cc) v += S[pass][rc][cc][id];
        }
        gram[(size_t)ch * 162 + e2] = v;
    }
}

int corr9_plan(int kh, int kw, int sh, int sw, int rh, int rw, int padding_same, int H, int W, int force_rb) {
    if (kh != 3 || kw != 3 || sh != 1 || sw != 1 || rh != 1 || rw != 1 || !padding_same) return 0;
    if (H < 6 || W < corr9::WC) return 0;
    if ((int64_t)H * W >= ((int64_t)1 << 28)) return 0;
    if ((force_rb == 8 || force_rb == 6 || force_rb == 4) && force_rb + 2 <= H) return force_rb;
    const int rows = H - 2;
    auto live = [&](int rb) { return (double)rows / (double)((rows + rb - 1) / rb * rb); };
    if (8 + 2 <= H && live(8) >= 0.85) return 8;
    int best = 0;
    double best_live = -1.0;
    const int cand[3] = {8, 6, 4};
    for (int i = 0; i < 3; ++i) {
        const int rb = cand[i];
        if (rb + 2 > H) continue;
        const double score = live(rb) - (rb == 4 ? 0.1 : 0.0);
        if (score > best_live + 1e-9) { best_live = score; best = rb; }
    }
    return best;
}

__global__ void __launch_bounds__(256)
corr9_pack_kernel(const float *__restrict__ act, int64_t n_valid, int hw, int64_t C, int64_t c_first, int n_ch, int G,
                  int64_t img0, int pix_per_warp, float *__restrict__ out) {
    const int lane = threadIdx.x & 31, VC = G * n_ch;
    const int64_t ng = blockIdx.y;
    const int p0 = (int)((blockIdx.x * (blockDim.x >> 5) + (threadIdx.x >> 5)) * pix_per_warp);
    const int p1 = min(hw, p0 + pix_per_warp);
    if (p0 >= p1) return;
    for (int vb = 0; vb < VC; vb += 32) {
        const int v = vb + lane;
        if (v >= VC) continue;
        const int g = v / n_ch, c = v - g * n_ch;
        const int64_t n = img0 + ng * G + g;
        float *dst = out + (ng * hw + p0) * VC + v;
        if (n < n_valid) {
            const float *src = act + (n * hw + p0) * C + c_first + c;
            int p = p0;
            for (; p + 8 <= p1; p += 8) {
                float t[8];
#pragma unroll
                for (int u = 0; u < 8; ++u) t[u] = __ldg(src + (int64_t)u * C);
#pragma unroll
                for (int u = 0; u < 8; ++u) dst[(int64_t)u * VC] = t[u];
                src += 8 * C;
                dst += (int64_t)8 * VC;
            }
            for (; p < p1; ++p) {
                *dst = __ldg(src);
                src += C;
                dst += VC;
            }
        } else {
            for (int p = p0; p < p1; ++p) {
                *dst = 0.f;
                dst += VC;
            }
        }
    }
}

int corr9_pack_stage(gpfq_ctx *ctx, const float *act, int64_t n_img, int H, int Wd, int64_t C, int64_t c_first, int n_ch, int G,
                     int64_t img0, int64_t imgs, float *out) {
    const int hw = H * Wd;
    const int64_t VC = (int64_t)G * n_ch, ngrp = ceil_div64(imgs, G);
    int64_t ppw = ceil_div64((int64_t)hw * ngrp, (int64_t)ctx->sm_count * 64);
    ppw = std::max<int64_t>(32, std::min<int64_t>(ppw, hw));
    const int64_t warps = ceil_div64(hw, ppw);
    for (int64_t g0 = 0; g0 < ngrp; g0 += 65535) {
        const int64_t gn = std::min<int64_t>(65535, ngrp - g0);
        dim3 grid((unsigned)ceil_div64(warps, 8), (unsigned)gn);
        corr9_pack_kernel<<<grid, 256, 0, ctx->stream>>>(act, std::min<int64_t>(n_img, img0 + imgs), hw, C, c_first, n_ch, G,
                                                         img0 + g0 * G, (int)ppw, out + (img0 / G + g0) * hw * VC);
        KERNEL_CHECK(ctx);
    }
    return GPFQ_OK;
}

template <int RB>
static int corr9_resident_ctas(bool same) {
    using namespace corr9;
    int a = 0, b = 0;
    if (cudaFuncSetAttribute(conv_corr9_tma_kernel<RB, false>, cudaFuncAttributeMaxDynamicSharedMemorySize, (int)Ring<RB, false>::SMEM) != cudaSuccess ||
        cudaOccupancyMaxActiveBlocksPerMultiprocessor(&a, conv_corr9_tma_kernel<RB, false>, WARPS * 32, Ring<RB, false>::SMEM) != cudaSuccess) {
        cudaGetLastError();
        return 0;
    }
    if (same) return a;
    if (cudaFuncSetAttribute(conv_corr9_tma_kernel<RB, true>, cudaFuncAttributeMaxDynamicSharedMemorySize, (int)Ring<RB, true>::SMEM) != cudaSuccess ||
        cudaOccupancyMaxActiveBlocksPerMultiprocessor(&b, conv_corr9_tma_kernel<RB, true>, WARPS * 32, Ring<RB, true>::SMEM) != cudaSuccess) {
        cudaGetLastError();
        return 0;
    }
    return a < b ? a : b;
}

static int corr9_strip_width(int Wd);
template <int SW, int RB>
static int corr9_strip_resident_ctas(bool same) {
    using namespace corr9s;
    int a = 0, b = 0;
    if (cudaFuncSetAttribute(conv_corr9_strip_kernel<SW, RB, false>, cudaFuncAttributeMaxDynamicSharedMemorySize, (int)Cfg<SW, RB, false>::SMEM) != cudaSuccess ||
        cudaOccupancyMaxActiveBlocksPerMultiprocessor(&a, conv_corr9_strip_kernel<SW, RB, false>, WARPS * 32, Cfg<SW, RB, false>::SMEM) != cudaSuccess) {
        cudaGetLastError();
        return 0;
    }
    if (same) return a;
    if (cudaFuncSetAttribute(conv_corr9_strip_kernel<SW, RB, true>, cudaFuncAttributeMaxDynamicSharedMemorySize, (int)Cfg<SW, RB, true>::SMEM) != cudaSuccess ||
        cudaOccupancyMaxActiveBlocksPerMultiprocessor(&b, conv_corr9_strip_kernel<SW, RB, true>, WARPS * 32, Cfg<SW, RB, true>::SMEM) != cudaSuccess) {
        cudaGetLastError();
        return 0;
    }
    return a < b ? a : b;
}

int corr9_pick_slots(gpfq_ctx *ctx, int RB, bool same, int64_t c_first, int n_ch, int64_t ntasks, int Wd) {
    using namespace corr9;
    if (RB < 1 || RB > 8) return WARPS;
    if (const int sw = ctx->corr_strip == 2 ? 0 : corr9_strip_width(Wd)) {
        const int rb = RB == 1 ? 1 : 4, wi = sw == 8 ? 0 : sw == 14 ? 1 : 2;
        int &socc = ctx->corr_strip_occ[same ? 1 : 0][rb == 1 ? 0 : 1][wi];
        if (!socc) {
            socc = rb == 1 ? (sw == 8 ? corr9_strip_resident_ctas<8, 1>(same) : sw == 14 ? corr9_strip_resident_ctas<14, 1>(same) : corr9_strip_resident_ctas<16, 1>(same))
                           : (sw == 8 ? corr9_strip_resident_ctas<8, 4>(same) : sw == 14 ? corr9_strip_resident_ctas<14, 4>(same) : corr9_strip_resident_ctas<16, 4>(same));
            if (socc < 1) socc = 1;
        }
        const int64_t groups = ceil_div64(n_ch + (c_first & 3), 32);
        int64_t ctas = std::max<int64_t>(1, (int64_t)ctx->sm_count * socc / groups);
        ctas = std::min<int64_t>(ctas, std::max<int64_t>(1, ceil_div64(ntasks, corr9s::WARPS)));
        return (int)(ctas * corr9s::WARPS);
    }
    int &occ = ctx->corr_occ[same ? 1 : 0][RB];
    if (!occ) {
        occ = RB == 8 ? corr9_resident_ctas<8>(same) : RB == 6 ? corr9_resident_ctas<6>(same)
              : RB == 4 ? corr9_resident_ctas<4>(same) : corr9_resident_ctas<1>(same);
        if (occ < 1) occ = 1;
    }
    const int64_t groups = ceil_div64(n_ch + (c_first & 3), 32);
    int64_t per = ceil_div64((int64_t)ctx->sm_count * occ * WARPS, groups);
    per = std::min<int64_t>(per, std::max<int64_t>(1, ntasks));
    return (int)(ceil_div64(per, WARPS) * WARPS);
}

typedef CUresult (*Corr9EncodeFn)(CUtensorMap *, CUtensorMapDataType, cuuint32_t, void *, const cuuint64_t *, const cuuint64_t *,
                                  const cuuint32_t *, const cuuint32_t *, CUtensorMapInterleave, CUtensorMapSwizzle,
                                  CUtensorMapL2promotion, CUtensorMapFloatOOBfill);

static Corr9EncodeFn corr9_encode_fn() {
    static Corr9EncodeFn fn = nullptr;
    if (!fn) {
        void *p = nullptr;
        cudaDriverEntryPointQueryResult q;
        if (cudaGetDriverEntryPoint("cuTensorMapEncodeTiled", &p, cudaEnableDefault, &q) == cudaSuccess && q == cudaDriverEntryPointSuccess)
            fn = reinterpret_cast<Corr9EncodeFn>(p);
    }
    return fn;
}

int corr9_tensor_ok(const float *act, const float *actq) {
    return corr9_encode_fn() != nullptr && ((uintptr_t)act & 15) == 0 && ((uintptr_t)actq & 15) == 0;
}

static bool corr9_make_map(CUtensorMap *map, const float *act, int64_t n_img_total, int H, int W, int64_t C, int rows,
                           int cols = corr9::WC) {
    Corr9EncodeFn enc = corr9_encode_fn();
    if (!enc) return false;
    const cuuint64_t dims[4] = {(cuuint64_t)C, (cuuint64_t)W, (cuuint64_t)H, (cuuint64_t)n_img_total};
    const cuuint64_t strides[3] = {(cuuint64_t)C * 4, (cuuint64_t)W * C * 4, (cuuint64_t)H * W * C * 4};
    const cuuint32_t box[4] = {32u, (cuuint32_t)cols, (cuuint32_t)rows, 1u};
    const cuuint32_t estr[4] = {1u, 1u, 1u, 1u};
    return enc(map, CU_TENSOR_MAP_DATA_TYPE_FLOAT32, 4, const_cast<float *>(act), dims, strides, box, estr,
               CU_TENSOR_MAP_INTERLEAVE_NONE, CU_TENSOR_MAP_SWIZZLE_NONE, CU_TENSOR_MAP_L2_PROMOTION_L2_128B,
               CU_TENSOR_MAP_FLOAT_OOB_FILL_NONE) == CUDA_SUCCESS;
}

template <int RB>
static int launch_corr9(gpfq_ctx *ctx, const float *actq, const float *actx, bool same, const Corr9Geom &gm, int64_t C,
                        int64_t n_img_total, double *partial, int slot_stride, int slot0) {
    using namespace corr9;
    cudaStream_t st = ctx->stream;
    dim3 grid((unsigned)(gm.slots / WARPS), (unsigned)ceil_div64(gm.n_ch + (gm.c_first & 3), 32));
    CUtensorMap mq_win, mq_ctr, mx_win;
    bool ok = corr9_make_map(&mq_win, actq, n_img_total, gm.H, gm.W, C, RB + 2);
    if (ok && !same)
        ok = corr9_make_map(&mq_ctr, actq, n_img_total, gm.H, gm.W, C, RB) &&
             corr9_make_map(&mx_win, actx, n_img_total, gm.H, gm.W, C, RB + 2);
    if (!ok) return gpfq_fail(ctx, GPFQ_ERR_CUDA, "cuTensorMapEncodeTiled failed for the (%lld, %d, %d, %lld) activations",
                              (long long)n_img_total, gm.H, gm.W, (long long)C);
    CUDA_TRY(ctx, cudaFuncSetAttribute(conv_corr9_tma_kernel<RB, false>, cudaFuncAttributeMaxDynamicSharedMemorySize,
                                       (int)Ring<RB, false>::SMEM));
    conv_corr9_tma_kernel<RB, false><<<grid, WARPS * 32, Ring<RB, false>::SMEM, st>>>(mq_win, mq_win, gm, partial, slot_stride, slot0);
    KERNEL_CHECK(ctx);
    if (!same) {
        CUDA_TRY(ctx, cudaFuncSetAttribute(conv_corr9_tma_kernel<RB, true>, cudaFuncAttributeMaxDynamicSharedMemorySize,
                                           (int)Ring<RB, true>::SMEM));
        conv_corr9_tma_kernel<RB, true><<<grid, WARPS * 32, Ring<RB, true>::SMEM, st>>>(mx_win, mq_ctr, gm, partial, slot_stride, slot0);
        KERNEL_CHECK(ctx);
    }
    return GPFQ_OK;
}


template <int SW, int RB>
static int launch_corr9_strip(gpfq_ctx *ctx, const float *actq, const float *actx, bool same, const Corr9Geom &gm, int64_t C,
                              int64_t n_img_total, double *partial, int slot_stride, int slot0) {
    using namespace corr9s;
    cudaStream_t st = ctx->stream;
    dim3 grid((unsigned)(gm.slots / WARPS), (unsigned)ceil_div64(gm.n_ch + (gm.c_first & 3), 32));
    CUtensorMap mq_win, mq_ctr, mx_win;
    bool ok = corr9_make_map(&mq_win, actq, n_img_total, gm.H, gm.W, C, RB + 2, SW + 4);
    if (ok && !same)
        ok = corr9_make_map(&mq_ctr, actq, n_img_total, gm.H, gm.W, C, RB, SW) &&
             corr9_make_map(&mx_win, actx, n_img_total, gm.H, gm.W, C, RB + 2, SW + 4);
    if (!ok) return gpfq_fail(ctx, GPFQ_ERR_CUDA, "cuTensorMapEncodeTiled failed for the (%lld, %d, %d, %lld) activations",
                              (long long)n_img_total, gm.H, gm.W, (long long)C);
    CUDA_TRY(ctx, cudaFuncSetAttribute(conv_corr9_strip_kernel<SW, RB, false>, cudaFuncAttributeMaxDynamicSharedMemorySize,
                                       (int)Cfg<SW, RB, false>::SMEM));
    conv_corr9_strip_kernel<SW, RB, false><<<grid, WARPS * 32, Cfg<SW, RB, false>::SMEM, st>>>(mq_win, mq_win, gm, partial, slot_stride, slot0);
    KERNEL_CHECK(ctx);
    if (!same) {
        CUDA_TRY(ctx, cudaFuncSetAttribute(conv_corr9_strip_kernel<SW, RB, true>, cudaFuncAttributeMaxDynamicSharedMemorySize,
                                           (int)Cfg<SW, RB, true>::SMEM));
        conv_corr9_strip_kernel<SW, RB, true><<<grid, WARPS * 32, Cfg<SW, RB, true>::SMEM, st>>>(mx_win, mq_ctr, gm, partial, slot_stride, slot0);
        KERNEL_CHECK(ctx);
    }
    return GPFQ_OK;
}

static int corr9_strip_width(int Wd) { return Wd == 8 ? 8 : (Wd == 14 || Wd == 28 || Wd == 56) ? 14 : (Wd == 16 || Wd == 32 || Wd == 64) ? 16 : 0; }

template <int SW>
static int corr9_strip_stage(gpfq_ctx *ctx, const float *actq, const float *act, bool same, Corr9Geom gm, int64_t C, int64_t n_img_total,
                             double *partial, int slot_stride, int slot0, int slots, double *rpartial, int rslot_stride, int rslot0,
                             int rslots) {
    if (gm.H > 2) {
        gm.slots = slots; gm.y_first = 1; gm.y_last = gm.H - 2; gm.two_rows = 0;
        GPFQ_TRY((launch_corr9_strip<SW, 4>(ctx, actq, act, same, gm, C, n_img_total, partial, slot_stride, slot0)));
    }
    gm.slots = rslots; gm.y_first = 0; gm.y_last = gm.H - 1; gm.two_rows = 1;
    GPFQ_TRY((launch_corr9_strip<SW, 1>(ctx, actq, act, same, gm, C, n_img_total, rpartial, rslot_stride, rslot0)));
    return GPFQ_OK;
}

int corr9_uses_strips(gpfq_ctx *ctx, int Wd) { return ctx->corr_strip != 2 && corr9_strip_width(Wd) != 0; }

int conv_corr9_stage(gpfq_ctx *ctx, const float *act, const float *actq, bool same, int64_t img0, int64_t n_img,
                     int64_t n_img_total, int H, int Wd, int64_t C, int64_t c_first, int n_ch, int RB, double *partial,
                     int slot_stride, int slot0, int slots, double *rpartial, int rslot_stride, int rslot0, int rslots) {
    using namespace corr9;
    if (slots % WARPS || rslots % WARPS || rslots < 2)
        return gpfq_fail(ctx, GPFQ_ERR_ARG, "corr9: slot counts must be multiples of %d", WARPS);
    if (n_img_total >= ((int64_t)1 << 31)) return gpfq_fail(ctx, GPFQ_ERR_ARG, "corr9: too many images");
    Corr9Geom gm;
    gm.H = H; gm.W = Wd; gm.c_first = c_first; gm.n_ch = n_ch; gm.img0 = img0; gm.n_img = n_img;
    if (const int sw = ctx->corr_strip == 2 ? 0 : corr9_strip_width(Wd)) {
        gm.slots = 0; gm.y_first = gm.y_last = gm.two_rows = 0;
        if (sw == 8) return corr9_strip_stage<8>(ctx, actq, act, same, gm, C, n_img_total, partial, slot_stride, slot0, slots, rpartial, rslot_stride, rslot0, rslots);
        if (sw == 14) return corr9_strip_stage<14>(ctx, actq, act, same, gm, C, n_img_total, partial, slot_stride, slot0, slots, rpartial, rslot_stride, rslot0, rslots);
        return corr9_strip_stage<16>(ctx, actq, act, same, gm, C, n_img_total, partial, slot_stride, slot0, slots, rpartial, rslot_stride, rslot0, rslots);
    }
    if (H > 2) {
        gm.slots = slots; gm.y_first = 1; gm.y_last = H - 2; gm.two_rows = 0;
        switch (RB) {
            case 8: GPFQ_TRY(launch_corr9<8>(ctx, actq, act, same, gm, C, n_img_total, partial, slot_stride, slot0)); break;
            case 6: GPFQ_TRY(launch_corr9<6>(ctx, actq, act, same, gm, C, n_img_total, partial, slot_stride, slot0)); break;
            case 4: GPFQ_TRY(launch_corr9<4>(ctx, actq, act, same, gm, C, n_img_total, partial, slot_stride, slot0)); break;
            default: return gpfq_fail(ctx, GPFQ_ERR_ARG, "corr9: no kernel for %d rows per band", RB);
        }
    }
    gm.slots = rslots; gm.y_first = 0; gm.y_last = H - 1; gm.two_rows = 1;
    GPFQ_TRY(launch_corr9<1>(ctx, actq, act, same, gm, C, n_img_total, rpartial, rslot_stride, rslot0));
    return GPFQ_OK;
}

__global__ void conv_corr9_sum_groups_kernel(const double *__restrict__ gv, int n_ch, int G, double *__restrict__ gram) {
    const int ch = blockIdx.x;
    for (int e = threadIdx.x; e < 162; e += blockDim.x) {
        double v = 0.0;
        for (int g = 0; g < G; ++g) v += gv[((size_t)g * n_ch + ch) * 162 + e];
        gram[(size_t)ch * 162 + e] = v;
    }
}

int conv_corr9_assemble_stage(gpfq_ctx *ctx, const double *partial, int slots, const double *rpartial, int rslots,
                              bool same, int n_ch, int G, double *gram) {
    if (G > 1) {
        double *gv = nullptr;
        GPFQ_TRY(gpfq_ws(ctx, WS_MISC, (size_t)G * n_ch * 162 * sizeof(double), (void **)&gv));
        conv_corr9_assemble_kernel<<<(unsigned)(G * n_ch), 1024, 0, ctx->stream>>>(partial, slots, rpartial, rslots, same ? 1 : 0,
                                                                                    G * n_ch, 1, gv);
        KERNEL_CHECK(ctx);
        conv_corr9_sum_groups_kernel<<<(unsigned)n_ch, 192, 0, ctx->stream>>>(gv, n_ch, G, gram);
        KERNEL_CHECK(ctx);
        return GPFQ_OK;
    }
    conv_corr9_assemble_kernel<<<(unsigned)n_ch, 1024, 0, ctx->stream>>>(partial, slots, rpartial, rslots, same ? 1 : 0, n_ch, G, gram);
    KERNEL_CHECK(ctx);
    return GPFQ_OK;
}
```

Baseline: 2.157 billion.

## Fuse the two corr9 passes into one kernel that reads both activations

When the quantized and original activations differ, the 3x3 conv correlation used to run two kernels, one for Q·Q and one for the X-vs-Q cross term, each streaming its own window. A single BOTH/one-pass kernel now loads a taller Q window plus the X centre rows once and accumulates both Gram blocks in separate registers. The cross term is computed from Q's perspective with mirrored offsets, and the assembly kernel gets a flag for the new layout. This removes one activation read and a kernel launch, at the cost of more registers and shared memory per warp, which may lower occupancy.

Result: faster. 2.269 billion (median of 6 runs) (+5.2%).

```diff
diff --git a/quantized_neural_networks_b200/csrc/api.cu b/quantized_neural_networks_b200/csrc/api.cu
--- a/quantized_neural_networks_b200/csrc/api.cu
+++ b/quantized_neural_networks_b200/csrc/api.cu
@@ -27,14 +27,14 @@
                  int, int, int, int, float *, int64_t);
 int msq_stage(gpfq_ctx *, const void *, int, int64_t, const double *, int, int, double *, const double *, int64_t);
 int nhwc9_plan(int, int, int, int, int, int, int, int, int *, int *);
-int corr9_plan(int, int, int, int, int, int, int, int, int, int);
+int corr9_plan(int, int, int, int, int, int, int, int, int, int, bool);
 int corr9_pack_stage(gpfq_ctx *, const float *, int64_t, int, int, int64_t, int64_t, int, int, int64_t, int64_t, float *);
 int corr9_pick_slots(gpfq_ctx *, int, bool, int64_t, int, int64_t, int);
 int corr9_uses_strips(gpfq_ctx *, int);
 int corr9_tensor_ok(const float *, const float *);
 int conv_corr9_stage(gpfq_ctx *, const float *, const float *, bool, int64_t, int64_t, int64_t, int, int, int64_t, int64_t, int,
                      int, double *, int, int, int, double *, int, int, int);
-int conv_corr9_assemble_stage(gpfq_ctx *, const double *, int, const double *, int, bool, int, int, double *);
+int conv_corr9_assemble_stage(gpfq_ctx *, const double *, int, const double *, int, bool, int, int, int, double *);
 int conv_gram9_nhwc_stage(gpfq_ctx *, const float *, const float *, bool, int64_t, int64_t, int, int, int64_t, int64_t, int,
                           int, int, int, int, int, int, int, double *, int);
 
@@ -1001,7 +1001,7 @@
         }
     }
     CUDA_TRY(ctx, gpfq_record(ctx, 5, s));
-    const int corr_rb = ctx->conv_variant == 0 ? corr9_plan(kh, kw, sh, sw, rh, rw, padding_same, (int)H, (int)Wd, ctx->corr_rb) : 0;
+    const int corr_rb = ctx->conv_variant == 0 ? corr9_plan(kh, kw, sh, sw, rh, rw, padding_same, (int)H, (int)Wd, ctx->corr_rb, same) : 0;
     const bool corr_direct = C >= 32 && C % 4 == 0 && n_ch >= 8 && (H * Wd >= 128 || (H * Wd >= 64 && corr9_uses_strips(ctx, (int)Wd)));
     int corr_G = 1;
     if (corr_rb && !(C >= 32 && C % 4 == 0) && (H * Wd >= 4096 || (H * Wd >= 1024 && corr9_uses_strips(ctx, (int)Wd))) && ctx->corr_pack != 2) {
@@ -1074,7 +1074,7 @@
                                           ic * per_ic, per_ic, bpartial, bslots, ic * bper_ic, bper_ic));
             }
         }
-        GPFQ_TRY(conv_corr9_assemble_stage(ctx, partial, slots, bpartial, bslots, same, (int)n_ch, pack ? corr_G : 1, gram));
+        GPFQ_TRY(conv_corr9_assemble_stage(ctx, partial, slots, bpartial, bslots, same, (int)Wd, (int)n_ch, pack ? corr_G : 1, gram));
         CUDA_TRY(ctx, gpfq_record(ctx, 3, s));
         GPFQ_TRY(conv_finish(ctx, kk, nullptr, (int)n_ch, 0, same, W, C, F, c0, al, n_alph, Q_out, flags, gram, groups, d_scales));
         CUDA_TRY(ctx, gpfq_record(ctx, 1, s));
diff --git a/quantized_neural_networks_b200/csrc/conv_corr.cu b/quantized_neural_networks_b200/csrc/conv_corr.cu
--- a/quantized_neural_networks_b200/csrc/conv_corr.cu
+++ b/quantized_neural_networks_b200/csrc/conv_corr.cu
@@ -41,24 +41,43 @@
             smem_u32(dst)), "l"(map), "r"(smem_u32(bar)), "r"(c), "r"(x), "r"(y), "r"(n)
         : "memory");
 }
-template <int RB, bool CROSS>
+template <int RB, bool BOTH>
 struct Ring {
-    static constexpr int NS = CROSS ? 2 : 3;
-    static constexpr int B_FLOATS = (RB + 2) * WC * 32;
-    static constexpr int A_FLOATS = CROSS ? RB * WC * 32 : 0;
+    static constexpr int NS = BOTH ? 2 : 3;
+    static constexpr int WR = BOTH ? RB + 4 : RB + 2;
+    static constexpr int B_FLOATS = WR * WC * 32;
+    static constexpr int A_FLOATS = BOTH ? RB * WC * 32 : 0;
     static constexpr int STAGE_FLOATS = B_FLOATS + A_FLOATS;
     static constexpr size_t WARP_BYTES = (size_t)NS * STAGE_FLOATS * sizeof(float);
     static constexpr size_t SMEM = WARPS * WARP_BYTES + WARPS * NS * sizeof(uint64_t);
 };
-}
-
-template <int RB, bool CROSS>
-__global__ void __launch_bounds__(corr9::WARPS * 32, RB <= 4 ? 3 : 2)
-conv_corr9_tma_kernel(const __grid_constant__ CUtensorMap mapB, const __grid_constant__ CUtensorMap mapA, Corr9Geom gm,
+template <int WR>
+__device__ __forceinline__ void mac_g2(double a, const double (&win)[WR][5], int i, int ph, double (&o)[ND]) {
+#pragma unroll
+    for (int dy = 0; dy < 2; ++dy)
+#pragma unroll
+        for (int dx = 0; dx < 5; ++dx) o[dy * 5 + dx] = fma(a, win[i + dy][(ph + 1 + dx) % 5], o[dy * 5 + dx]);
+#pragma unroll
+    for (int dx = 0; dx < 3; ++dx) o[10 + dx] = fma(a, win[i + 2][(ph + 1 + dx) % 5], o[10 + dx]);
+}
+template <int WR>
+__device__ __forceinline__ void mac_g1(double a, const double (&win)[WR][5], int i, int ph, double (&o)[ND]) {
+#pragma unroll
+    for (int dy = 0; dy < 2; ++dy)
+#pragma unroll
+        for (int dx = 0; dx < 5; ++dx) o[dy * 5 + dx] = fma(a, win[i + 4 - dy][(ph + 5 - dx) % 5], o[dy * 5 + dx]);
+#pragma unroll
+    for (int dx = 0; dx < 3; ++dx) o[10 + dx] = fma(a, win[i + 2][(ph + 5 - dx) % 5], o[10 + dx]);
+}
+}
+
+template <int RB, bool BOTH>
+__global__ void __launch_bounds__(corr9::WARPS * 32, (RB <= 4 && !BOTH) || RB == 1 ? 3 : 2)
+conv_corr9_tma_kernel(const __grid_constant__ CUtensorMap mapQ, const __grid_constant__ CUtensorMap mapX, Corr9Geom gm,
                       double *__restrict__ partial, int slot_stride, int slot0) {
     using namespace corr9;
-    using R = Ring<RB, CROSS>;
-    constexpr int NS = R::NS;
+    using R = Ring<RB, BOTH>;
+    constexpr int NS = R::NS, WR = R::WR;
     extern __shared__ __align__(128) unsigned char corr9_smem[];
     const int lane = threadIdx.x & 31, warp = threadIdx.x >> 5;
     const int slot = blockIdx.x * WARPS + warp;
@@ -79,11 +98,11 @@
     const int64_t ntasks = gm.two_rows ? gm.n_img : gm.n_img * nbands;
     const int64_t t_first = gm.two_rows ? slot / 2 : slot, t_step = gm.two_rows ? gm.slots / 2 : gm.slots;
     const int nstages = (W + 2 + WC - 1) / WC;
-    double *rec = partial + ((size_t)(chok ? chl : 0) * slot_stride + slot0 + slot) * REC + (CROSS ? 0 : 3 * ND);
+    double *rec = partial + ((size_t)(chok ? chl : 0) * slot_stride + slot0 + slot) * REC;
     uint32_t it = 0;
-    double acc[ND];
-#pragma unroll
-    for (int d = 0; d < ND; ++d) acc[d] = 0.0;
+    double acc[ND], acc1[ND];
+#pragma unroll
+    for (int d = 0; d < ND; ++d) acc[d] = acc1[d] = 0.0;
 
     const int step_img = (int)(gm.two_rows ? t_step : t_step / nbands), step_band = gm.two_rows ? 0 : (int)(t_step % nbands);
     const int img_first = (int)(gm.img0 + (gm.two_rows ? t_first : t_first / nbands));
@@ -99,8 +118,8 @@
                 const int s = (int)(ppos % NS);
                 float *dst = ring + s * R::STAGE_FLOATS;
                 mbar_expect_tx(&bars[s], (uint32_t)(R::STAGE_FLOATS * sizeof(float)));
-                tma_load_4d(dst, &mapB, &bars[s], c0, pk * WC, py0 - 2, pimg);
-                if (CROSS) tma_load_4d(dst + R::B_FLOATS, &mapA, &bars[s], c0, pk * WC - 2, py0, pimg);
+                tma_load_4d(dst, &mapQ, &bars[s], c0, pk * WC, py0 - 2, pimg);
+                if (BOTH) tma_load_4d(dst + R::B_FLOATS, &mapX, &bars[s], c0, pk * WC - 2, py0, pimg);
             }
             ++ppos;
             if (++pk == nstages) {
@@ -124,11 +143,11 @@
 #pragma unroll
         for (int i = 0; i < RB; ++i) rowmask |= (y0 + i <= gm.y_last) ? (1u << i) : 0u;
         const bool allrows = rowmask == (1u << RB) - 1u;
-        double win[RB + 2][5];
+        double win[WR][5];
         double ac[RB];
         (void)ac;
 #pragma unroll
-        for (int r = 0; r < RB + 2; ++r)
+        for (int r = 0; r < WR; ++r)
 #pragma unroll
             for (int c = 0; c < 5; ++c) win[r][c] = 0.0;
         for (int k = 0; k < nstages; ++k) {
@@ -143,31 +162,24 @@
 #pragma unroll
                 for (int ph = 0; ph < WC; ++ph) {
 #pragma unroll
-                    for (int r = 0; r < RB + 2; ++r) win[r][ph] = (double)tb[(r * WC + ph) * 32];
-                    if (CROSS) {
+                    for (int r = 0; r < WR; ++r) win[r][ph] = (double)tb[(r * WC + ph) * 32];
+                    if (BOTH) {
 #pragma unroll
                         for (int i = 0; i < RB; ++i) ac[i] = (double)ta[(i * WC + ph) * 32];
                     }
 #pragma unroll
                     for (int i = 0; i < RB; ++i) {
-                        const double a = CROSS ? ac[i] : win[i + 2][(ph + 3) % 5];
-#pragma unroll
-                        for (int dy = 0; dy < 2; ++dy)
-#pragma unroll
-                            for (int dx = 0; dx < 5; ++dx)
-                                acc[dy * 5 + dx] = fma(a, win[i + dy][(ph + 1 + dx) % 5], acc[dy * 5 + dx]);
-#pragma unroll
-                        for (int dx = 0; dx < 3; ++dx)
-                            acc[10 + dx] = fma(a, win[i + 2][(ph + 1 + dx) % 5], acc[10 + dx]);
+                        mac_g2(win[i + 2][(ph + 3) % 5], win, i, ph, acc);
+                        if (BOTH) mac_g1(ac[i], win, i, ph, acc1);
                     }
                 }
             } else {
-                float rawb[RB + 2], rawa[RB];
+                float rawb[WR], rawa[RB];
                 (void)rawa;
                 auto fetch = [&](int ph) {
 #pragma unroll
-                    for (int r = 0; r < RB + 2; ++r) rawb[r] = tb[(r * WC + ph) * 32];
-                    if (CROSS) {
+                    for (int r = 0; r < WR; ++r) rawb[r] = tb[(r * WC + ph) * 32];
+                    if (BOTH) {
 #pragma unroll
                         for (int i = 0; i < RB; ++i) rawa[i] = ta[(i * WC + ph) * 32];
                     }
@@ -178,38 +190,38 @@
                     const int cx = k * WC + ph;
                     if (cx < W + 2) {
 #pragma unroll
-                        for (int r = 0; r < RB + 2; ++r) win[r][ph] = (double)rawb[r];
-                        if (CROSS) {
+                        for (int r = 0; r < WR; ++r) win[r][ph] = (double)rawb[r];
+                        if (BOTH) {
 #pragma unroll
                             for (int i = 0; i < RB; ++i) ac[i] = (double)rawa[i];
                         }
                         if (ph + 1 < WC) fetch(ph + 1);
                         if (cx >= 2) {
-                            double e[ND];
-#pragma unroll
-                            for (int d = 0; d < ND; ++d) e[d] = 0.0;
-#pragma unroll
-                            for (int i = 0; i < RB; ++i) {
-                                double a = CROSS ? ac[i] : win[i + 2][(ph + 3) % 5];
-                                a = (rowmask >> i) & 1u ? a : 0.0;
-#pragma unroll
-                                for (int dy = 0; dy < 2; ++dy)
-#pragma unroll
-                                    for (int dx = 0; dx < 5; ++dx)
-                                        e[dy * 5 + dx] = fma(a, win[i + dy][(ph + 1 + dx) % 5], e[dy * 5 + dx]);
-#pragma unroll
-                                for (int dx = 0; dx < 3; ++dx)
-                                    e[10 + dx] = fma(a, win[i + 2][(ph + 1 + dx) % 5], e[10 + dx]);
-                            }
-                            if (cx == 2 || cx == W + 1) {
-                                if (chok) {
-                                    double *o = rec + (cx == 2 ? 0 : 2 * ND);
-#pragma unroll
-                                    for (int d = 0; d < ND; ++d) atomicAdd(o + d, e[d]);
+                            const bool edge = cx == 2 || cx == W + 1;
+                            double *o = rec + (cx == 2 ? 0 : 2 * ND);
+#pragma unroll
+                            for (int pass = BOTH ? 0 : 1; pass < 2; ++pass) {
+                                double e[ND];
+#pragma unroll
+                                for (int d = 0; d < ND; ++d) e[d] = 0.0;
+#pragma unroll
+                                for (int i = 0; i < RB; ++i) {
+                                    const bool live = (rowmask >> i) & 1u;
+                                    if (pass == 1) mac_g2(live ? win[i + 2][(ph + 3) % 5] : 0.0, win, i, ph, e);
+                                    else mac_g1(live ? ac[i] : 0.0, win, i, ph, e);
                                 }
-                            } else {
-#pragma unroll
-                                for (int d = 0; d < ND; ++d) acc[d] += e[d];
+                                if (edge) {
+                                    if (chok) {
+#pragma unroll
+                                        for (int d = 0; d < ND; ++d) atomicAdd(o + pass * 3 * ND + d, e[d]);
+                                    }
+                                } else if (pass == 1) {
+#pragma unroll
+                                    for (int d = 0; d < ND; ++d) acc[d] += e[d];
+                                } else {
+#pragma unroll
+                                    for (int d = 0; d < ND; ++d) acc1[d] += e[d];
+                                }
                             }
                         }
                     }
@@ -220,7 +232,10 @@
     }
     if (chok) {
 #pragma unroll
-        for (int d = 0; d < ND; ++d) rec[ND + d] = acc[d];
+        for (int d = 0; d < ND; ++d) {
+            rec[3 * ND + ND + d] = acc[d];
+            if (BOTH) rec[ND + d] = acc1[d];
+        }
     }
 }
 
@@ -385,9 +400,171 @@
     }
 }
 
+namespace corr9s {
+template <int SW, int RB>
+struct Cfg1 {
+    static constexpr int BW = SW + 4, WR = RB + 4;
+    static constexpr int WIN_FLOATS = WR * BW * 32;
+    static constexpr int CTR_FLOATS = RB * SW * 32;
+    static constexpr int STAGE_FLOATS = WIN_FLOATS + CTR_FLOATS;
+    static constexpr int NS = Boxes<RB>::NS;
+    static constexpr size_t WARP_BYTES = (size_t)NS * STAGE_FLOATS * sizeof(float);
+    static constexpr size_t REC_BYTES = (size_t)2 * 2 * ND * 32 * sizeof(double);
+    static constexpr size_t SMEM = WARPS * (WARP_BYTES + REC_BYTES) + WARPS * NS * sizeof(uint64_t);
+};
+}
+
+template <int SW, int RB>
+__global__ void __launch_bounds__(corr9s::WARPS * 32)
+conv_corr9_strip1_kernel(const __grid_constant__ CUtensorMap mapQ, const __grid_constant__ CUtensorMap mapX, Corr9Geom gm,
+                         double *__restrict__ partial, int slot_stride, int slot0) {
+    using namespace corr9s;
+    using corr9::mbar_expect_tx;
+    using corr9::mbar_init;
+    using corr9::mbar_wait;
+    using corr9::tma_load_4d;
+    using C = Cfg1<SW, RB>;
+    constexpr int BW = C::BW, WR = C::WR, NS = C::NS;
+    extern __shared__ __align__(128) unsigned char corr9_smem[];
+    const int lane = threadIdx.x & 31, warp = threadIdx.x >> 5;
+    const int slot = blockIdx.x * WARPS + warp;
+    const int c0 = (int)(gm.c_first & ~(int64_t)3) + (int)blockIdx.y * 32;
+    const int chl = c0 + lane - (int)gm.c_first;
+    const bool chok = chl >= 0 && chl < gm.n_ch;
+    float *ring = reinterpret_cast<float *>(corr9_smem + warp * C::WARP_BYTES);
+    double *srec = reinterpret_cast<double *>(corr9_smem + WARPS * C::WARP_BYTES + warp * C::REC_BYTES) + lane;
+    uint64_t *bars = reinterpret_cast<uint64_t *>(corr9_smem + WARPS * (C::WARP_BYTES + C::REC_BYTES)) + warp * NS;
+#pragma unroll
+    for (int j = 0; j < 4 * ND; ++j) srec[j * 32] = 0.0;
+    if (lane == 0) {
+#pragma unroll
+        for (int s = 0; s < NS; ++s) mbar_init(&bars[s], 1);
+        asm volatile("fence.mbarrier_init.release.cluster;\n" ::: "memory");
+    }
+    __syncwarp();
+    const int nstrips = gm.W / SW;
+    const int nrows = gm.y_last - gm.y_first + 1;
+    const int nbands = gm.two_rows ? 1 : (nrows + RB - 1) / RB;
+    const int per_img = nbands * nstrips;
+    const int64_t ntasks = gm.n_img * per_img;
+    const int64_t t_first = gm.two_rows ? slot / 2 : slot, t_step = gm.two_rows ? gm.slots / 2 : gm.slots;
+    const int row_fixed = (slot & 1) ? gm.y_last : gm.y_first;
+    const int step_img = (int)(t_step / per_img), step_in = (int)(t_step % per_img);
+    auto fetch = [&](int img, int in, uint32_t pos) {
+        const int band = in / nstrips, strip = in - band * nstrips;
+        const int y0 = gm.two_rows ? row_fixed : gm.y_first + band * RB, x0 = strip * SW;
+        const int s = (int)(pos % NS);
+        float *dst = ring + s * C::STAGE_FLOATS;
+        mbar_expect_tx(&bars[s], (uint32_t)(C::STAGE_FLOATS * sizeof(float)));
+        tma_load_4d(dst, &mapQ, &bars[s], c0, x0 - 2, y0 - 2, img);
+        tma_load_4d(dst + C::WIN_FLOATS, &mapX, &bars[s], c0, x0, y0, img);
+    };
+    double acc1[ND], acc2[ND];
+#pragma unroll
+    for (int d = 0; d < ND; ++d) acc1[d] = acc2[d] = 0.0;
+    int img = (int)(gm.img0 + t_first / per_img), in = (int)(t_first % per_img);
+    if (t_first < ntasks && lane == 0) fetch(img, in, 0);
+    uint32_t pos = 0;
+    for (int64_t task = t_first; task < ntasks; task += t_step, ++pos) {
+        int nimg = img + step_img, nin = in + step_in;
+        if (nin >= per_img) { nin -= per_img; ++nimg; }
+        if (NS > 1) {
+            __syncwarp();
+            if (task + t_step < ntasks && lane == 0) fetch(nimg, nin, pos + 1);
+        }
+        const int band = in / nstrips, strip = in - band * nstrips;
+        const int y0 = gm.two_rows ? row_fixed : gm.y_first + band * RB;
+        const bool left_edge = strip == 0, right_edge = strip == nstrips - 1;
+        unsigned rowmask = 0;
+#pragma unroll
+        for (int i = 0; i < RB; ++i) rowmask |= (y0 + i <= gm.y_last) ? (1u << i) : 0u;
+        const int s = (int)(pos % NS);
+        mbar_wait(&bars[s], (pos / NS) & 1u);
+        const float *tb = ring + s * C::STAGE_FLOATS + lane;
+        const float *ta = tb + C::WIN_FLOATS;
+        double win[WR][6];
+        double ctr[RB], ctr_n[RB];
+#pragma unroll
+        for (int bc = 0; bc < 5; ++bc)
+#pragma unroll
+            for (int r = 0; r < WR; ++r) win[r][bc] = (double)tb[(r * BW + bc) * 32];
+#pragma unroll
+        for (int i = 0; i < RB; ++i) ctr[i] = (double)ta[(i * SW) * 32];
+#pragma unroll
+        for (int p = 0; p < SW; ++p) {
+            const bool edge = p == 0 || p == SW - 1;
+            double e1[ND], e2[ND];
+            if (edge) {
+#pragma unroll
+                for (int d = 0; d < ND; ++d) e1[d] = e2[d] = 0.0;
+            }
+#pragma unroll
+            for (int i = 0; i < RB; ++i) {
+                const bool live = (rowmask >> i) & 1u;
+                const double q = live ? win[i + 2][(p + 2) % 6] : 0.0, xc = live ? ctr[i] : 0.0;
+                double *o1 = edge ? e1 : acc1, *o2 = edge ? e2 : acc2;
+#pragma unroll
+                for (int dy = 0; dy < 2; ++dy)
+#pragma unroll
+                    for (int dx = 0; dx < 5; ++dx) {
+                        o2[dy * 5 + dx] = fma(q, win[i + dy][(p + dx) % 6], o2[dy * 5 + dx]);
+                        o1[dy * 5 + dx] = fma(xc, win[i + 4 - dy][(p + 4 - dx) % 6], o1[dy * 5 + dx]);
+                    }
+#pragma unroll
+                for (int dx = 0; dx < 3; ++dx) {
+                    o2[10 + dx] = fma(q, win[i + 2][(p + dx) % 6], o2[10 + dx]);
+                    o1[10 + dx] = fma(xc, win[i + 2][(p + 4 - dx) % 6], o1[10 + dx]);
+                }
+                if (p + 5 < BW) {
+#pragma unroll
+                    for (int r = i; r < WR; r += RB) win[r][(p + 5) % 6] = (double)tb[(r * BW + p + 5) * 32];
+                }
+                if (p + 1 < SW) ctr_n[i] = (double)ta[(i * SW + p + 1) * 32];
+            }
+#pragma unroll
+            for (int i = 0; i < RB; ++i) ctr[i] = ctr_n[i];
+            if (edge) {
+                const bool first = p == 0 && left_edge, last = p == SW - 1 && right_edge;
+                if (first || last) {
+                    double *r = srec + (last ? 2 * ND * 32 : 0);
+#pragma unroll
+                    for (int d = 0; d < ND; ++d) {
+                        r[d * 32] += e1[d];
+                        r[(ND + d) * 32] += e2[d];
+                    }
+                } else {
+#pragma unroll
+                    for (int d = 0; d < ND; ++d) {
+                        acc1[d] += e1[d];
+                        acc2[d] += e2[d];
+                    }
+                }
+            }
+        }
+        if (NS == 1) {
+            __syncwarp();
+            if (task + t_step < ntasks && lane == 0) fetch(nimg, nin, pos + 1);
+        }
+        img = nimg;
+        in = nin;
+    }
+    if (chok) {
+        double *rec = partial + ((size_t)chl * slot_stride + slot0 + slot) * REC;
+#pragma unroll
+        for (int d = 0; d < ND; ++d) {
+            rec[d] = srec[d * 32];
+            rec[ND + d] = acc1[d];
+            rec[2 * ND + d] = srec[(2 * ND + d) * 32];
+            rec[3 * ND + d] = srec[(ND + d) * 32];
+            rec[4 * ND + d] = acc2[d];
+            rec[5 * ND + d] = srec[(3 * ND + d) * 32];
+        }
+    }
+}
+
 __global__ void __launch_bounds__(1024)
 conv_corr9_assemble_kernel(const double *__restrict__ partial, int slots, const double *__restrict__ rpartial, int rslots,
-                           int same, int n_ch, int G, double *__restrict__ gram) {
+                           int same, int g1_by_x, int n_ch, int G, double *__restrict__ gram) {
     using namespace corr9;
     constexpr int NV = 2 * 9 * ND, NP = 4;
     __shared__ double S[2][3][3][ND];
@@ -433,7 +610,9 @@
             const int ar = t / 3, ac = t % 3, dy = s / 3 - ar, dx = s % 3 - ac;
             const int id = dy < 0 ? (dy + 2) * 5 + dx + 2 : 12 + dx;
             const int pass = (which == 0 && !same) ? 0 : 1;
-            const int r_lo = ar == 2 ? 1 : 0, r_hi = ar == 0 ? 1 : 2, c_lo = ac == 2 ? 1 : 0, c_hi = ac == 0 ? 1 : 2;
+            const bool by_s = pass == 0 && g1_by_x;
+            const int cr = by_s ? s / 3 : ar, ccl = by_s ? s % 3 : ac;
+            const int r_lo = cr == 2 ? 1 : 0, r_hi = cr == 0 ? 1 : 2, c_lo = ccl == 2 ? 1 : 0, c_hi = ccl == 0 ? 1 : 2;
             for (int rc = r_lo; rc <= r_hi; ++rc)
                 for (int cc = c_lo; cc <= c_hi; ++cc) v += S[pass][rc][cc][id];
         }
@@ -441,11 +620,16 @@
     }
 }
 
-int corr9_plan(int kh, int kw, int sh, int sw, int rh, int rw, int padding_same, int H, int W, int force_rb) {
+int corr9_plan(int kh, int kw, int sh, int sw, int rh, int rw, int padding_same, int H, int W, int force_rb, bool same) {
     if (kh != 3 || kw != 3 || sh != 1 || sw != 1 || rh != 1 || rw != 1 || !padding_same) return 0;
     if (H < 6 || W < corr9::WC) return 0;
     if ((int64_t)H * W >= ((int64_t)1 << 28)) return 0;
-    if ((force_rb == 8 || force_rb == 6 || force_rb == 4) && force_rb + 2 <= H) return force_rb;
+    if ((force_rb == 8 || force_rb == 6 || force_rb == 4) && force_rb + 2 <= H && (same || force_rb != 8)) return force_rb;
+    if (!same) {
+        const int rows = H - 2;
+        const int bands6 = (rows + 5) / 6, bands4 = (rows + 3) / 4;
+        return 6 + 2 <= H && ((double)rows >= 0.85 * bands6 * 6 || bands6 * 6 <= bands4 * 4) ? 6 : 4;
+    }
     const int rows = H - 2;
     auto live = [&](int rb) { return (double)rows / (double)((rows + rb - 1) / rb * rb); };
     if (8 + 2 <= H && live(8) >= 0.85) return 8;
@@ -518,41 +702,50 @@
     return GPFQ_OK;
 }
 
-template <int RB>
-static int corr9_resident_ctas(bool same) {
+template <int RB, bool BOTH>
+static int corr9_resident_ctas() {
     using namespace corr9;
-    int a = 0, b = 0;
-    if (cudaFuncSetAttribute(conv_corr9_tma_kernel<RB, false>, cudaFuncAttributeMaxDynamicSharedMemorySize, (int)Ring<RB, false>::SMEM) != cudaSuccess ||
-        cudaOccupancyMaxActiveBlocksPerMultiprocessor(&a, conv_corr9_tma_kernel<RB, false>, WARPS * 32, Ring<RB, false>::SMEM) != cudaSuccess) {
+    int a = 0;
+    if (cudaFuncSetAttribute(conv_corr9_tma_kernel<RB, BOTH>, cudaFuncAttributeMaxDynamicSharedMemorySize, (int)Ring<RB, BOTH>::SMEM) != cudaSuccess ||
+        cudaOccupancyMaxActiveBlocksPerMultiprocessor(&a, conv_corr9_tma_kernel<RB, BOTH>, WARPS * 32, Ring<RB, BOTH>::SMEM) != cudaSuccess) {
         cudaGetLastError();
         return 0;
     }
-    if (same) return a;
-    if (cudaFuncSetAttribute(conv_corr9_tma_kernel<RB, true>, cudaFuncAttributeMaxDynamicSharedMemorySize, (int)Ring<RB, true>::SMEM) != cudaSuccess ||
-        cudaOccupancyMaxActiveBlocksPerMultiprocessor(&b, conv_corr9_tma_kernel<RB, true>, WARPS * 32, Ring<RB, true>::SMEM) != cudaSuccess) {
-        cudaGetLastError();
-        return 0;
-    }
-    return a < b ? a : b;
-}
-
+    return a;
+}
+
+static constexpr bool corr9_strip_onepass_sw(int sw) { return sw == 8; }
 static int corr9_strip_width(int Wd);
+static bool corr9_strip_onepass(int Wd);
 template <int SW, int RB>
 static int corr9_strip_resident_ctas(bool same) {
     using namespace corr9s;
     int a = 0, b = 0;
+    if constexpr (corr9_strip_onepass_sw(SW)) {
+        if (!same) {
+            if (cudaFuncSetAttribute(conv_corr9_strip1_kernel<SW, RB>, cudaFuncAttributeMaxDynamicSharedMemorySize, (int)Cfg1<SW, RB>::SMEM) != cudaSuccess ||
+                cudaOccupancyMaxActiveBlocksPerMultiprocessor(&a, conv_corr9_strip1_kernel<SW, RB>, WARPS * 32, Cfg1<SW, RB>::SMEM) != cudaSuccess) {
+                cudaGetLastError();
+                return 0;
+            }
+            return a;
+        }
+    }
     if (cudaFuncSetAttribute(conv_corr9_strip_kernel<SW, RB, false>, cudaFuncAttributeMaxDynamicSharedMemorySize, (int)Cfg<SW, RB, false>::SMEM) != cudaSuccess ||
         cudaOccupancyMaxActiveBlocksPerMultiprocessor(&a, conv_corr9_strip_kernel<SW, RB, false>, WARPS * 32, Cfg<SW, RB, false>::SMEM) != cudaSuccess) {
         cudaGetLastError();
         return 0;
     }
-    if (same) return a;
-    if (cudaFuncSetAttribute(conv_corr9_strip_kernel<SW, RB, true>, cudaFuncAttributeMaxDynamicSharedMemorySize, (int)Cfg<SW, RB, true>::SMEM) != cudaSuccess ||
-        cudaOccupancyMaxActiveBlocksPerMultiprocessor(&b, conv_corr9_strip_kernel<SW, RB, true>, WARPS * 32, Cfg<SW, RB, true>::SMEM) != cudaSuccess) {
-        cudaGetLastError();
-        return 0;
-    }
-    return a < b ? a : b;
+    if constexpr (!corr9_strip_onepass_sw(SW)) {
+        if (same) return a;
+        if (cudaFuncSetAttribute(conv_corr9_strip_kernel<SW, RB, true>, cudaFuncAttributeMaxDynamicSharedMemorySize, (int)Cfg<SW, RB, true>::SMEM) != cudaSuccess ||
+            cudaOccupancyMaxActiveBlocksPerMultiprocessor(&b, conv_corr9_strip_kernel<SW, RB, true>, WARPS * 32, Cfg<SW, RB, true>::SMEM) != cudaSuccess) {
+            cudaGetLastError();
+            return 0;
+        }
+        return a < b ? a : b;
+    }
+    return a;
 }
 
 int corr9_pick_slots(gpfq_ctx *ctx, int RB, bool same, int64_t c_first, int n_ch, int64_t ntasks, int Wd) {
@@ -573,8 +766,9 @@
     }
     int &occ = ctx->corr_occ[same ? 1 : 0][RB];
     if (!occ) {
-        occ = RB == 8 ? corr9_resident_ctas<8>(same) : RB == 6 ? corr9_resident_ctas<6>(same)
-              : RB == 4 ? corr9_resident_ctas<4>(same) : corr9_resident_ctas<1>(same);
+        occ = same ? (RB == 8 ? corr9_resident_ctas<8, false>() : RB == 6 ? corr9_resident_ctas<6, false>()
+                      : RB == 4 ? corr9_resident_ctas<4, false>() : corr9_resident_ctas<1, false>())
+                   : (RB == 6 ? corr9_resident_ctas<6, true>() : RB == 4 ? corr9_resident_ctas<4, true>() : corr9_resident_ctas<1, true>());
         if (occ < 1) occ = 1;
     }
     const int64_t groups = ceil_div64(n_ch + (c_first & 3), 32);
@@ -615,29 +809,20 @@
                CU_TENSOR_MAP_FLOAT_OOB_FILL_NONE) == CUDA_SUCCESS;
 }
 
-template <int RB>
-static int launch_corr9(gpfq_ctx *ctx, const float *actq, const float *actx, bool same, const Corr9Geom &gm, int64_t C,
-                        int64_t n_img_total, double *partial, int slot_stride, int slot0) {
+template <int RB, bool BOTH>
+static int launch_corr9(gpfq_ctx *ctx, const float *actq, const float *actx, const Corr9Geom &gm, int64_t C, int64_t n_img_total,
+                        double *partial, int slot_stride, int slot0) {
     using namespace corr9;
-    cudaStream_t st = ctx->stream;
+    using R = Ring<RB, BOTH>;
     dim3 grid((unsigned)(gm.slots / WARPS), (unsigned)ceil_div64(gm.n_ch + (gm.c_first & 3), 32));
-    CUtensorMap mq_win, mq_ctr, mx_win;
-    bool ok = corr9_make_map(&mq_win, actq, n_img_total, gm.H, gm.W, C, RB + 2);
-    if (ok && !same)
-        ok = corr9_make_map(&mq_ctr, actq, n_img_total, gm.H, gm.W, C, RB) &&
-             corr9_make_map(&mx_win, actx, n_img_total, gm.H, gm.W, C, RB + 2);
+    CUtensorMap mq_win, mx_ctr;
+    bool ok = corr9_make_map(&mq_win, actq, n_img_total, gm.H, gm.W, C, R::WR);
+    if (ok && BOTH) ok = corr9_make_map(&mx_ctr, actx, n_img_total, gm.H, gm.W, C, RB);
     if (!ok) return gpfq_fail(ctx, GPFQ_ERR_CUDA, "cuTensorMapEncodeTiled failed for the (%lld, %d, %d, %lld) activations",
                               (long long)n_img_total, gm.H, gm.W, (long long)C);
-    CUDA_TRY(ctx, cudaFuncSetAttribute(conv_corr9_tma_kernel<RB, false>, cudaFuncAttributeMaxDynamicSharedMemorySize,
-                                       (int)Ring<RB, false>::SMEM));
-    conv_corr9_tma_kernel<RB, false><<<grid, WARPS * 32, Ring<RB, false>::SMEM, st>>>(mq_win, mq_win, gm, partial, slot_stride, slot0);
+    CUDA_TRY(ctx, cudaFuncSetAttribute(conv_corr9_tma_kernel<RB, BOTH>, cudaFuncAttributeMaxDynamicSharedMemorySize, (int)R::SMEM));
+    conv_corr9_tma_kernel<RB, BOTH><<<grid, WARPS * 32, R::SMEM, ctx->stream>>>(mq_win, BOTH ? mx_ctr : mq_win, gm, partial, slot_stride, slot0);
     KERNEL_CHECK(ctx);
-    if (!same) {
-        CUDA_TRY(ctx, cudaFuncSetAttribute(conv_corr9_tma_kernel<RB, true>, cudaFuncAttributeMaxDynamicSharedMemorySize,
-                                           (int)Ring<RB, true>::SMEM));
-        conv_corr9_tma_kernel<RB, true><<<grid, WARPS * 32, Ring<RB, true>::SMEM, st>>>(mx_win, mq_ctr, gm, partial, slot_stride, slot0);
-        KERNEL_CHECK(ctx);
-    }
     return GPFQ_OK;
 }
 
@@ -649,6 +834,19 @@
     cudaStream_t st = ctx->stream;
     dim3 grid((unsigned)(gm.slots / WARPS), (unsigned)ceil_div64(gm.n_ch + (gm.c_first & 3), 32));
     CUtensorMap mq_win, mq_ctr, mx_win;
+    if constexpr (corr9_strip_onepass_sw(SW)) {
+        if (!same) {
+        using C1 = Cfg1<SW, RB>;
+        if (!corr9_make_map(&mq_win, actq, n_img_total, gm.H, gm.W, C, C1::WR, SW + 4) ||
+            !corr9_make_map(&mq_ctr, actx, n_img_total, gm.H, gm.W, C, RB, SW))
+            return gpfq_fail(ctx, GPFQ_ERR_CUDA, "cuTensorMapEncodeTiled failed for the (%lld, %d, %d, %lld) activations",
+                             (long long)n_img_total, gm.H, gm.W, (long long)C);
+        CUDA_TRY(ctx, cudaFuncSetAttribute(conv_corr9_strip1_kernel<SW, RB>, cudaFuncAttributeMaxDynamicSharedMemorySize, (int)C1::SMEM));
+        conv_corr9_strip1_kernel<SW, RB><<<grid, WARPS * 32, C1::SMEM, st>>>(mq_win, mq_ctr, gm, partial, slot_stride, slot0);
+        KERNEL_CHECK(ctx);
+        return GPFQ_OK;
+        }
+    }
     bool ok = corr9_make_map(&mq_win, actq, n_img_total, gm.H, gm.W, C, RB + 2, SW + 4);
     if (ok && !same)
         ok = corr9_make_map(&mq_ctr, actq, n_img_total, gm.H, gm.W, C, RB, SW) &&
@@ -659,16 +857,19 @@
                                        (int)Cfg<SW, RB, false>::SMEM));
     conv_corr9_strip_kernel<SW, RB, false><<<grid, WARPS * 32, Cfg<SW, RB, false>::SMEM, st>>>(mq_win, mq_win, gm, partial, slot_stride, slot0);
     KERNEL_CHECK(ctx);
-    if (!same) {
-        CUDA_TRY(ctx, cudaFuncSetAttribute(conv_corr9_strip_kernel<SW, RB, true>, cudaFuncAttributeMaxDynamicSharedMemorySize,
-                                           (int)Cfg<SW, RB, true>::SMEM));
-        conv_corr9_strip_kernel<SW, RB, true><<<grid, WARPS * 32, Cfg<SW, RB, true>::SMEM, st>>>(mx_win, mq_ctr, gm, partial, slot_stride, slot0);
-        KERNEL_CHECK(ctx);
+    if constexpr (!corr9_strip_onepass_sw(SW)) {
+        if (!same) {
+            CUDA_TRY(ctx, cudaFuncSetAttribute(conv_corr9_strip_kernel<SW, RB, true>, cudaFuncAttributeMaxDynamicSharedMemorySize,
+                                               (int)Cfg<SW, RB, true>::SMEM));
+            conv_corr9_strip_kernel<SW, RB, true><<<grid, WARPS * 32, Cfg<SW, RB, true>::SMEM, st>>>(mx_win, mq_ctr, gm, partial, slot_stride, slot0);
+            KERNEL_CHECK(ctx);
+        }
     }
     return GPFQ_OK;
 }
 
 static int corr9_strip_width(int Wd) { return Wd == 8 ? 8 : (Wd == 14 || Wd == 28 || Wd == 56) ? 14 : (Wd == 16 || Wd == 32 || Wd == 64) ? 16 : 0; }
+static bool corr9_strip_onepass(int Wd) { return corr9_strip_onepass_sw(corr9_strip_width(Wd)); }
 
 template <int SW>
 static int corr9_strip_stage(gpfq_ctx *ctx, const float *actq, const float *act, bool same, Corr9Geom gm, int64_t C, int64_t n_img_total,
@@ -702,15 +903,19 @@
     }
     if (H > 2) {
         gm.slots = slots; gm.y_first = 1; gm.y_last = H - 2; gm.two_rows = 0;
-        switch (RB) {
-            case 8: GPFQ_TRY(launch_corr9<8>(ctx, actq, act, same, gm, C, n_img_total, partial, slot_stride, slot0)); break;
-            case 6: GPFQ_TRY(launch_corr9<6>(ctx, actq, act, same, gm, C, n_img_total, partial, slot_stride, slot0)); break;
-            case 4: GPFQ_TRY(launch_corr9<4>(ctx, actq, act, same, gm, C, n_img_total, partial, slot_stride, slot0)); break;
-            default: return gpfq_fail(ctx, GPFQ_ERR_ARG, "corr9: no kernel for %d rows per band", RB);
+        const int rc = same ? RB : -RB;
+        switch (rc) {
+            case 8: GPFQ_TRY((launch_corr9<8, false>(ctx, actq, act, gm, C, n_img_total, partial, slot_stride, slot0))); break;
+            case 6: GPFQ_TRY((launch_corr9<6, false>(ctx, actq, act, gm, C, n_img_total, partial, slot_stride, slot0))); break;
+            case 4: GPFQ_TRY((launch_corr9<4, false>(ctx, actq, act, gm, C, n_img_total, partial, slot_stride, slot0))); break;
+            case -6: GPFQ_TRY((launch_corr9<6, true>(ctx, actq, act, gm, C, n_img_total, partial, slot_stride, slot0))); break;
+            case -4: GPFQ_TRY((launch_corr9<4, true>(ctx, actq, act, gm, C, n_img_total, partial, slot_stride, slot0))); break;
+            default: return gpfq_fail(ctx, GPFQ_ERR_ARG, "corr9: no kernel for %d rows per band (X~ %s X)", RB, same ? "==" : "!=");
         }
     }
     gm.slots = rslots; gm.y_first = 0; gm.y_last = H - 1; gm.two_rows = 1;
-    GPFQ_TRY(launch_corr9<1>(ctx, actq, act, same, gm, C, n_img_total, rpartial, rslot_stride, rslot0));
+    if (same) GPFQ_TRY((launch_corr9<1, false>(ctx, actq, act, gm, C, n_img_total, rpartial, rslot_stride, rslot0)));
+    else GPFQ_TRY((launch_corr9<1, true>(ctx, actq, act, gm, C, n_img_total, rpartial, rslot_stride, rslot0)));
     return GPFQ_OK;
 }
 
@@ -724,18 +929,19 @@
 }
 
 int conv_corr9_assemble_stage(gpfq_ctx *ctx, const double *partial, int slots, const double *rpartial, int rslots,
-                              bool same, int n_ch, int G, double *gram) {
+                              bool same, int Wd, int n_ch, int G, double *gram) {
+    const int g1_by_x = corr9_uses_strips(ctx, Wd) && !corr9_strip_onepass(Wd) ? 0 : 1;
     if (G > 1) {
         double *gv = nullptr;
         GPFQ_TRY(gpfq_ws(ctx, WS_MISC, (size_t)G * n_ch * 162 * sizeof(double), (void **)&gv));
         conv_corr9_assemble_kernel<<<(unsigned)(G * n_ch), 1024, 0, ctx->stream>>>(partial, slots, rpartial, rslots, same ? 1 : 0,
-                                                                                    G * n_ch, 1, gv);
+                                                                                    g1_by_x, G * n_ch, 1, gv);
         KERNEL_CHECK(ctx);
         conv_corr9_sum_groups_kernel<<<(unsigned)n_ch, 192, 0, ctx->stream>>>(gv, n_ch, G, gram);
         KERNEL_CHECK(ctx);
         return GPFQ_OK;
     }
-    conv_corr9_assemble_kernel<<<(unsigned)n_ch, 1024, 0, ctx->stream>>>(partial, slots, rpartial, rslots, same ? 1 : 0, n_ch, G, gram);
+    conv_corr9_assemble_kernel<<<(unsigned)n_ch, 1024, 0, ctx->stream>>>(partial, slots, rpartial, rslots, same ? 1 : 0, g1_by_x, n_ch, G, gram);
     KERNEL_CHECK(ctx);
     return GPFQ_OK;
 }
```
